# kiliant/zklaim

Hardware: AMD Instinct MI355X
Metric: Groth16 proofs/sec (zklaim gadget, alt_bn128) + G1 MSM GB/s vs HBM roofline (higher is better)
Workload: dtype u32 limbs, Montgomery (254-bit Fq/Fr: 9 x 29-bit in the accumulation, reduction and NTT kernels, 8 x 32-bit elsewhere)

## Files before the change

zklaim_amd/csrc/msm.hip:

```cpp
#include "common.hpp"
#include "fq29.hip.hpp"
#include "../../include/zkg.h"
#include <algorithm>
#include <chrono>
#include <cstdio>
#include <cstdlib>
#include <cstring>
#include <mutex>

#define ZK_VGPR_CAP(n) __attribute__((amdgpu_num_vgpr((n) / 2)))
static constexpr int ACC29_VGPRS = 192;

namespace zk {

static constexpr int SCALAR_BITS = 255;
template <class F> struct RedGeom { static constexpr int LANES_LOG = sizeof(F) == sizeof(Fq) ? 7 : 6, LANES = 1 << LANES_LOG, THREADS = 4 * LANES; };
static constexpr int RED_L_LOG_TINY = 0, RED_L_LOG_SMALL = 2, RED_L_LOG_LARGE = 4;
static constexpr size_t RED_SMALL_BUCKETS = (size_t)1 << 16, RED_LARGE_BUCKETS = (size_t)1 << 18;
static constexpr int MAX_C = 16;
static constexpr uint32_t HEAVY_S = 512;
static constexpr uint32_t HEAVY_T_MAX = 1024;
static constexpr int HEAVY_PART_BLOCKS = 512, HEAVY_MERGE_BLOCKS = 128;
static constexpr int SORT_THREADS = 1024;
static constexpr int SCAN_ITEMS = 4;

struct MsmGeom { uint32_t c, W, B, Wt, w0, ws; };
struct SetLayout { size_t buckets, items, heavy, partials, folded, red_out; };
template <class F> struct BaseView {
    const Affine<F> *p; size_t level_stride; const uint32_t *gather; uint32_t index_sub, B; const uint32_t *remap;
    template <bool PLAIN = false> ZK_D Affine<F> load(uint32_t e, size_t gb) const {
        if constexpr (PLAIN) return p[e >> 1];
        uint32_t i = e >> 1;
        if (gather) i = gather[i];
        if (remap) i = remap[i];
        if (i < index_sub) return Affine<F>::inf();
        return p[(level_stride ? (gb / B) * level_stride : 0) + (i - index_sub)];
    }
};
template <class F> struct ViewSet { BaseView<F> v[MSM_MAX_SETS]; };
struct HeavyItem { uint32_t start, end, gb, single; };
struct HeavyBucket { uint32_t gb, first_item, nparts; };

static MsmGeom pick_geom(size_t n, int window_hint, uint32_t w0 = 0, uint32_t ws = 1) {
    int lg = 0; while (((size_t)1 << (lg + 1)) <= n) ++lg;
    int c = lg >= 15 ? 16 : lg >= 11 ? 12 : lg + 1;
    if (c < 4) c = 4;
    if (window_hint > 0) c = window_hint;
    static const char *force = getenv("ZKG_MSM_C");
    if (force && atoi(force) >= 2) c = atoi(force);
    if (c > MAX_C) c = MAX_C;
    MsmGeom g; g.c = c; g.Wt = (SCALAR_BITS + c - 1) / c; g.B = 1u << (c - 1);
    g.w0 = w0; g.ws = ws ? ws : 1; g.W = w0 < g.Wt ? (g.Wt - w0 + g.ws - 1) / g.ws : 0;
    return g;
}

ZK_D uint32_t bits_at(const uint32_t v[8], uint32_t off, uint32_t c) {
    uint32_t limb = off >> 5, sh = off & 31;
    if (limb >= 8) return 0;
    uint64_t x = v[limb];
    if (limb + 1 < 8) x |= (uint64_t)v[limb + 1] << 32;
    return (uint32_t)(x >> sh) & ((1u << c) - 1);
}

ZK_D void sort_wave_priority() { __builtin_amdgcn_s_setprio(3); }


struct ZeroList { uint32_t *p[4]; uint32_t words[4]; };
__global__ __launch_bounds__(256) void k_digits(const uint32_t *scalars, const uint32_t *gather, size_t n, int mont, MsmGeom g, uint32_t *digits, ZeroList zl) {
    sort_wave_priority();
    size_t i = (size_t)blockIdx.x * blockDim.x + threadIdx.x;
    const size_t lanes = (size_t)gridDim.x * blockDim.x;
#pragma unroll
    for (int k = 0; k < 4; ++k) for (size_t z = i; z < zl.words[k]; z += lanes) zl.p[k][z] = 0;
    if (i >= n) return;
    Fr f;
    const uint4 *p = reinterpret_cast<const uint4 *>(scalars + 8 * (gather ? (size_t)gather[i] : i));
    uint4 a = p[0], b = p[1];
    f.v[0] = a.x; f.v[1] = a.y; f.v[2] = a.z; f.v[3] = a.w; f.v[4] = b.x; f.v[5] = b.y; f.v[6] = b.z; f.v[7] = b.w;
    if (mont) f = f.from_mont();
    uint32_t carry = 0;
    for (uint32_t w = 0, own = g.w0, slot = 0; w < g.Wt; ++w) {
        uint32_t raw = bits_at(f.v, w * g.c, g.c) + carry, code = 0;
        if (raw > g.B) { uint32_t d = (1u << g.c) - raw; carry = 1; if (d) code = (d << 1) | 1u; }
        else { carry = 0; if (raw) code = raw << 1; }
        if (w == own) { digits[(size_t)slot * n + i] = code; ++slot; own += g.ws; }
    }
}

template <int C>
__global__ __launch_bounds__(256) void k_digits_c(const uint32_t *scalars, const uint32_t *gather, size_t n, int mont, MsmGeom g, uint32_t *digits, ZeroList zl) {
    sort_wave_priority();
    size_t i = (size_t)blockIdx.x * blockDim.x + threadIdx.x;
    const size_t lanes = (size_t)gridDim.x * blockDim.x;
#pragma unroll
    for (int k = 0; k < 4; ++k) for (size_t z = i; z < zl.words[k]; z += lanes) zl.p[k][z] = 0;
    if (i >= n) return;
    Fr f;
    const uint4 *p = reinterpret_cast<const uint4 *>(scalars + 8 * (gather ? (size_t)gather[i] : i));
    uint4 a = p[0], b = p[1];
    f.v[0] = a.x; f.v[1] = a.y; f.v[2] = a.z; f.v[3] = a.w; f.v[4] = b.x; f.v[5] = b.y; f.v[6] = b.z; f.v[7] = b.w;
    if (mont) f = f.from_mont();
    constexpr int WT = (SCALAR_BITS + C - 1) / C;
    constexpr uint32_t B = 1u << (C - 1), MASK = (1u << C) - 1;
    uint32_t carry = 0, own = g.w0, slot = 0;
#pragma unroll
    for (int w = 0; w < WT; ++w) {
        const int off = w * C, limb = off >> 5, sh = off & 31;
        uint32_t v = limb < 8 ? f.v[limb < 8 ? limb : 7] >> sh : 0u;
        if (sh + C > 32 && limb + 1 < 8) v |= f.v[limb + 1 < 8 ? limb + 1 : 7] << (32 - sh);
        const uint32_t raw = (v & MASK) + carry;
        const bool neg = raw > B;
        const uint32_t d = neg ? (1u << C) - raw : raw;
        carry = neg ? 1u : 0u;
        const uint32_t code = d ? (d << 1) | (neg ? 1u : 0u) : 0u;
        if ((uint32_t)w == own) { digits[(size_t)slot * n + i] = code; ++slot; own += g.ws; }
    }
}

template <int C>
__global__ __launch_bounds__(256) void k_digits_multi(const uint32_t *scalars, size_t scalar_stride , size_t n, int mont, uint32_t merge, uint32_t *digits, ZeroList zl) {
    sort_wave_priority();
    size_t i = (size_t)blockIdx.x * blockDim.x + threadIdx.x;
    const size_t lanes = (size_t)gridDim.x * blockDim.x;
    if (blockIdx.y == 0) {
#pragma unroll
        for (int k = 0; k < 4; ++k) for (size_t z = i; z < zl.words[k]; z += lanes) zl.p[k][z] = 0;
    }
    if (i >= n) return;
    const uint32_t p = blockIdx.y, P = gridDim.y;
    Fr f;
    const uint4 *src = reinterpret_cast<const uint4 *>(scalars + (size_t)p * scalar_stride + 8 * i);
    uint4 a = src[0], b = src[1];
    f.v[0] = a.x; f.v[1] = a.y; f.v[2] = a.z; f.v[3] = a.w; f.v[4] = b.x; f.v[5] = b.y; f.v[6] = b.z; f.v[7] = b.w;
    if (mont) f = f.from_mont();
    constexpr int WT = (SCALAR_BITS + C - 1) / C;
    constexpr uint32_t B = 1u << (C - 1), MASK = (1u << C) - 1;
    uint32_t carry = 0;
#pragma unroll
    for (int w = 0; w < WT; ++w) {
        const int off = w * C, limb = off >> 5, sh = off & 31;
        uint32_t v = limb < 8 ? f.v[limb < 8 ? limb : 7] >> sh : 0u;
        if (sh + C > 32 && limb + 1 < 8) v |= f.v[limb + 1 < 8 ? limb + 1 : 7] << (32 - sh);
        const uint32_t raw = (v & MASK) + carry;
        const bool neg = raw > B;
        const uint32_t d = neg ? (1u << C) - raw : raw;
        carry = neg ? 1u : 0u;
        const uint32_t code = d ? (d << 1) | (neg ? 1u : 0u) : 0u;
        const size_t row = ((size_t)((uint32_t)w / merge) * P + p) * merge + (uint32_t)w % merge;
        digits[row * n + i] = code;
    }
}

__global__ __launch_bounds__(256) void k_digits_multi_any(const uint32_t *scalars, size_t scalar_stride, size_t n, int mont, MsmGeom g, uint32_t merge, uint32_t *digits, ZeroList zl) {
    sort_wave_priority();
    size_t i = (size_t)blockIdx.x * blockDim.x + threadIdx.x;
    const size_t lanes = (size_t)gridDim.x * blockDim.x;
    if (blockIdx.y == 0) {
#pragma unroll
        for (int k = 0; k < 4; ++k) for (size_t z = i; z < zl.words[k]; z += lanes) zl.p[k][z] = 0;
    }
    if (i >= n) return;
    const uint32_t p = blockIdx.y, P = gridDim.y;
    Fr f;
    const uint4 *src = reinterpret_cast<const uint4 *>(scalars + (size_t)p * scalar_stride + 8 * i);
    uint4 a = src[0], b = src[1];
    f.v[0] = a.x; f.v[1] = a.y; f.v[2] = a.z; f.v[3] = a.w; f.v[4] = b.x; f.v[5] = b.y; f.v[6] = b.z; f.v[7] = b.w;
    if (mont) f = f.from_mont();
    uint32_t carry = 0;
    for (uint32_t w = 0; w < g.Wt; ++w) {
        uint32_t raw = bits_at(f.v, w * g.c, g.c) + carry, code = 0;
        if (raw > g.B) { uint32_t d = (1u << g.c) - raw; carry = 1; if (d) code = (d << 1) | 1u; }
        else { carry = 0; if (raw) code = raw << 1; }
        const size_t row = ((size_t)(w / merge) * P + p) * merge + w % merge;
        digits[row * n + i] = code;
    }
}

template <int C>
__global__ __launch_bounds__(256) void k_digits_c4(const uint32_t *scalars, size_t n, int mont, MsmGeom g, uint32_t *digits, ZeroList zl) {
    sort_wave_priority();
    size_t i = (size_t)blockIdx.x * blockDim.x + threadIdx.x;
    const size_t lanes = (size_t)gridDim.x * blockDim.x;
#pragma unroll
    for (int k = 0; k < 4; ++k) for (size_t z = i; z < zl.words[k]; z += lanes) zl.p[k][z] = 0;
    if (4 * i >= n) return;
    Fr f[4];
#pragma unroll
    for (int q = 0; q < 4; ++q) {
        const uint4 *p = reinterpret_cast<const uint4 *>(scalars + 8 * (4 * i + q));
        const uint4 a = p[0], b = p[1];
        f[q].v[0] = a.x; f[q].v[1] = a.y; f[q].v[2] = a.z; f[q].v[3] = a.w; f[q].v[4] = b.x; f[q].v[5] = b.y; f[q].v[6] = b.z; f[q].v[7] = b.w;
        if (mont) f[q] = f[q].from_mont();
    }
    constexpr int WT = (SCALAR_BITS + C - 1) / C;
    constexpr uint32_t B = 1u << (C - 1), MASK = (1u << C) - 1;
    uint32_t carry[4] = {0, 0, 0, 0};
#pragma unroll
    for (int w = 0; w < WT; ++w) {
        const int off = w * C, limb = off >> 5, sh = off & 31;
        uint32_t code[4];
#pragma unroll
        for (int q = 0; q < 4; ++q) {
            uint32_t v = limb < 8 ? f[q].v[limb < 8 ? limb : 7] >> sh : 0u;
            if (sh + C > 32 && limb + 1 < 8) v |= f[q].v[limb + 1 < 8 ? limb + 1 : 7] << (32 - sh);
            const uint32_t raw = (v & MASK) + carry[q];
            const bool neg = raw > B;
            const uint32_t d = neg ? (1u << C) - raw : raw;
            carry[q] = neg ? 1u : 0u;
            code[q] = d ? (d << 1) | (neg ? 1u : 0u) : 0u;
        }
        *reinterpret_cast<uint4 *>(digits + (size_t)w * n + 4 * i) = make_uint4(code[0], code[1], code[2], code[3]);
    }
}

__global__ __launch_bounds__(SORT_THREADS) void k_hist(const uint32_t *digits, size_t n, uint32_t B, uint32_t S, uint32_t slice_len, uint32_t *hist) {
    extern __shared__ uint32_t lds_u32[];
    const uint32_t s = blockIdx.x, w = blockIdx.y, t = threadIdx.x;
    for (uint32_t b = t; b < B; b += SORT_THREADS) lds_u32[b] = 0;
    __syncthreads();
    size_t lo = (size_t)s * slice_len, hi = lo + slice_len < n ? lo + slice_len : n;
    const uint32_t *d = digits + (size_t)w * n;
    for (size_t i = lo + t; i < hi; i += SORT_THREADS) { uint32_t code = d[i]; if (code) atomicAdd(&lds_u32[(code >> 1) - 1], 1u); }
    __syncthreads();
    uint32_t *out = hist + ((size_t)w * S + s) * B;
    for (uint32_t b = t; b < B; b += SORT_THREADS) out[b] = lds_u32[b];
}

__global__ __launch_bounds__(256) void k_colscan(uint32_t *hist, uint32_t B, uint32_t S, size_t total, uint32_t *counts) {
    size_t gb = (size_t)blockIdx.x * blockDim.x + threadIdx.x;
    if (gb >= total) return;
    uint32_t w = (uint32_t)(gb / B), b = (uint32_t)(gb % B), run = 0;
    uint32_t *col = hist + (size_t)w * S * B + b;
    for (uint32_t s = 0; s < S; ++s) { uint32_t v = col[(size_t)s * B]; col[(size_t)s * B] = run; run += v; }
    counts[gb] = run;
}

__global__ __launch_bounds__(1024) void k_scan_blocks(const uint32_t *in, uint32_t *out, uint32_t *sums, size_t total) {
    __shared__ uint32_t part[1024];
    const uint32_t t = threadIdx.x;
    size_t base = ((size_t)blockIdx.x * 1024 + t) * SCAN_ITEMS;
    uint32_t v[SCAN_ITEMS], s = 0;
    for (int j = 0; j < SCAN_ITEMS; ++j) { v[j] = base + j < total ? in[base + j] : 0; s += v[j]; }
    part[t] = s;
    __syncthreads();
    for (uint32_t d = 1; d < 1024; d <<= 1) {
        uint32_t x = (t >= d) ? part[t - d] : 0;
        __syncthreads();
        part[t] += x;
        __syncthreads();
    }
    uint32_t run = part[t] - s;
    for (int j = 0; j < SCAN_ITEMS; ++j) { if (base + j < total) out[base + j] = run; run += v[j]; }
    if (t == 1023) sums[blockIdx.x] = part[1023];
}
__global__ __launch_bounds__(1024) void k_scan_sums(uint32_t *sums, uint32_t nblk, uint32_t *grand_total) {
    __shared__ uint32_t part[1024];
    const uint32_t t = threadIdx.x;
    uint32_t s = t < nblk ? sums[t] : 0;
    part[t] = s;
    __syncthreads();
    for (uint32_t d = 1; d < 1024; d <<= 1) {
        uint32_t x = (t >= d) ? part[t - d] : 0;
        __syncthreads();
        part[t] += x;
        __syncthreads();
    }
    if (t < nblk) sums[t] = part[t] - s;
    if (t == 1023) *grand_total = part[1023];
}
__global__ __launch_bounds__(1024) void k_scan_apply(uint32_t *out, const uint32_t *sums, size_t total) {
    size_t base = ((size_t)blockIdx.x * 1024 + threadIdx.x) * SCAN_ITEMS;
    uint32_t add = sums[blockIdx.x];
    for (int j = 0; j < SCAN_ITEMS; ++j) if (base + j < total) out[base + j] += add;
}

__global__ __launch_bounds__(SORT_THREADS) void k_place(const uint32_t *digits, size_t n, uint32_t B, uint32_t S, uint32_t slice_len,
                                                         const uint32_t *hist, const uint32_t *offsets, uint32_t *sorted) {
    extern __shared__ uint32_t lds_u32[];
    const uint32_t s = blockIdx.x, w = blockIdx.y, t = threadIdx.x;
    const uint32_t *rel = hist + ((size_t)w * S + s) * B, *off = offsets + (size_t)w * B;
    for (uint32_t b = t; b < B; b += SORT_THREADS) lds_u32[b] = off[b] + rel[b];
    __syncthreads();
    size_t lo = (size_t)s * slice_len, hi = lo + slice_len < n ? lo + slice_len : n;
    const uint32_t *d = digits + (size_t)w * n;
    for (size_t i = lo + t; i < hi; i += SORT_THREADS) {
        uint32_t code = d[i];
        if (code) { uint32_t pos = atomicAdd(&lds_u32[(code >> 1) - 1], 1u); sorted[pos] = ((uint32_t)i << 1) | (code & 1u); }
    }
}


static constexpr uint32_t RX_MAX_CBITS = 10, RX_MAX_CB = 1u << RX_MAX_CBITS, RX_SLICE = 16384, RX_PER_THREAD = 16, RX_FINE_MAX = 8192, RX_BIN_AVG = 4096;
__global__ __launch_bounds__(1024) void k_rx_count(const uint32_t *digits, size_t n, uint32_t fbits, uint32_t cbits, uint32_t *cnt) {
    sort_wave_priority();
    __shared__ uint32_t c[RX_MAX_CB];
    const uint32_t sl = blockIdx.x, w = blockIdx.y, t = threadIdx.x, CB = 1u << cbits;
    if (t < CB) c[t] = 0;
    __syncthreads();
    size_t lo = (size_t)sl * RX_SLICE, hi = lo + RX_SLICE < n ? lo + RX_SLICE : n;
    const uint32_t *d = digits + (size_t)w * n;
    if ((n & 3) == 0) {
        for (size_t i = lo + 4 * t; i < hi; i += 4096) {
            const uint4 q = *reinterpret_cast<const uint4 *>(d + i);
            if (q.x) atomicAdd(&c[((q.x >> 1) - 1) >> fbits], 1u);
            if (q.y) atomicAdd(&c[((q.y >> 1) - 1) >> fbits], 1u);
            if (q.z) atomicAdd(&c[((q.z >> 1) - 1) >> fbits], 1u);
            if (q.w) atomicAdd(&c[((q.w >> 1) - 1) >> fbits], 1u);
        }
    } else
    for (size_t i = lo + t; i < hi; i += 1024) { uint32_t code = d[i]; if (code) atomicAdd(&c[((code >> 1) - 1) >> fbits], 1u); }
    __syncthreads();
    if (t < CB && c[t]) atomicAdd(&cnt[w * CB + t], c[t]);
}
__global__ __launch_bounds__(1024) void k_rx_scan(const uint32_t *cnt, uint32_t nbins, uint32_t *base, uint32_t *cursor, uint32_t *grand_total) {
    sort_wave_priority();
    __shared__ uint32_t part[1024];
    const uint32_t t = threadIdx.x, per = (nbins + 1023) / 1024, lo = t * per, hi = lo + per < nbins ? lo + per : nbins;
    uint32_t sum = 0;
    for (uint32_t i = lo; i < hi; ++i) sum += cnt[i];
    part[t] = sum;
    __syncthreads();
    for (uint32_t d = 1; d < 1024; d <<= 1) {
        uint32_t x = (t >= d) ? part[t - d] : 0;
        __syncthreads();
        part[t] += x;
        __syncthreads();
    }
    uint32_t run = part[t] - sum;
    for (uint32_t i = lo; i < hi; ++i) { base[i] = run; cursor[i] = 0; run += cnt[i]; }
    if (t == 1023) { base[nbins] = part[1023]; *grand_total = part[1023]; }
}
template <int T>
__global__ __launch_bounds__(T) void k_rx_scatter(const uint32_t *digits, size_t n, uint32_t fbits, uint32_t cbits, const uint32_t *base, uint32_t *cursor,
                                                   uint32_t *tmp) {
    sort_wave_priority();
    extern __shared__ uint32_t lds_u32[];
    constexpr uint32_t SLICE = RX_PER_THREAD * T;
    const uint32_t CB = 1u << cbits;
    uint32_t *stage = lds_u32, *c = lds_u32 + SLICE, *off = c + RX_MAX_CB, *gb = off + RX_MAX_CB + 1, *cur = gb + RX_MAX_CB;
    const uint32_t sl = blockIdx.x, w = blockIdx.y, t = threadIdx.x;
    for (uint32_t b = t; b < CB; b += T) c[b] = 0;
    __syncthreads();
    size_t lo = (size_t)sl * SLICE, hi = lo + SLICE < n ? lo + SLICE : n;
    const uint32_t *d = digits + (size_t)w * n;
    uint32_t code[RX_PER_THREAD];
    const bool vec = (n & 3) == 0;
    auto elem = [&](uint32_t j) -> size_t { return vec ? lo + 4 * (size_t)t + (size_t)(j >> 2) * (4 * T) + (j & 3) : lo + t + (size_t)j * T; };
    if (vec) {
#pragma unroll
        for (uint32_t j = 0; j < RX_PER_THREAD; j += 4) {
            const size_t i = elem(j);
            uint4 q = make_uint4(0, 0, 0, 0);
            if (i < hi) q = *reinterpret_cast<const uint4 *>(d + i);
            code[j] = q.x; code[j + 1] = q.y; code[j + 2] = q.z; code[j + 3] = q.w;
        }
    } else {
#pragma unroll
        for (uint32_t j = 0; j < RX_PER_THREAD; ++j) { const size_t i = elem(j); code[j] = i < hi ? d[i] : 0; }
    }
#pragma unroll
    for (uint32_t j = 0; j < RX_PER_THREAD; ++j) if (code[j]) atomicAdd(&c[((code[j] >> 1) - 1) >> fbits], 1u);
    __syncthreads();
    const uint32_t b0 = t, b1 = t + T;
    if (b0 < CB) off[b0] = c[b0];
    if (b1 < CB) off[b1] = c[b1];
    __syncthreads();
    for (uint32_t dd = 1; dd < CB; dd <<= 1) {
        const uint32_t x0 = (b0 < CB && b0 >= dd) ? off[b0 - dd] : 0, x1 = (b1 < CB && b1 >= dd) ? off[b1 - dd] : 0;
        __syncthreads();
        if (b0 < CB) off[b0] += x0;
        if (b1 < CB) off[b1] += x1;
        __syncthreads();
    }
    if (t == 0) off[CB] = off[CB - 1];
    __syncthreads();
    for (uint32_t b = t; b < CB; b += T) { off[b] -= c[b]; gb[b] = c[b] ? base[w * CB + b] + atomicAdd(&cursor[w * CB + b], c[b]) : 0; cur[b] = 0; }
    __syncthreads();
    const uint32_t fmask = (1u << fbits) - 1;
#pragma unroll
    for (uint32_t j = 0; j < RX_PER_THREAD; ++j) {
        if (!code[j]) continue;
        uint32_t i = (uint32_t)elem(j), b = (code[j] >> 1) - 1, k = b >> fbits;
        uint32_t pos = off[k] + atomicAdd(&cur[k], 1u);
        stage[pos] = ((b & fmask) << (32 - fbits)) | (i << 1) | (code[j] & 1u);
    }
    __syncthreads();
    const uint32_t wave = t >> 6, lane = t & 63;
    for (uint32_t k = wave; k < CB; k += T / 64) {
        const uint32_t a = off[k], b = off[k + 1], g = gb[k];
        for (uint32_t p = a + lane; p < b; p += 64) tmp[g + (p - a)] = stage[p];
    }
}
ZK_D void rx_fine_offsets(uint32_t *cf, uint32_t *of, uint32_t FB, uint32_t t, uint32_t start, size_t gb0, uint32_t *counts, uint32_t *offsets) {
    const uint32_t T = blockDim.x;
    if (t < FB) of[t] = cf[t];
    __syncthreads();
    for (uint32_t d = 1; d < FB; d <<= 1) {
        uint32_t x = (t < FB && t >= d) ? of[t - d] : 0;
        __syncthreads();
        if (t < FB) of[t] += x;
        __syncthreads();
    }
    if (t < FB) of[t] -= cf[t];
    __syncthreads();
    for (uint32_t f = t; f < FB; f += T) { counts[gb0 + f] = cf[f]; offsets[gb0 + f] = start + of[f]; }
}
ZK_D void rx_fine_big_bin(const uint32_t *tmp, uint32_t fbits, uint32_t start, uint32_t cnt, size_t gb0, uint32_t *cf, uint32_t *of, uint32_t *cur, uint32_t *counts,
                          uint32_t *offsets, uint32_t *sorted) {
    const uint32_t FB = 1u << fbits, sh = 32 - fbits, low = (1u << sh) - 1, t = threadIdx.x, T = blockDim.x;
    const bool giant = cnt > 8 * RX_FINE_MAX;
    if (!giant) {
        for (uint32_t p = t; p < cnt; p += T) atomicAdd(&cf[tmp[start + p] >> sh], 1u);
    } else
    for (uint32_t p0 = 0; p0 < cnt; p0 += T) {
        uint32_t p = p0 + t; bool live = p < cnt; uint32_t f = live ? tmp[start + p] >> sh : 0;
        while (__any(live)) {
            uint32_t lf = __shfl(f, __ffsll((long long)__ballot(live)) - 1, 64);
            unsigned long long same = __ballot(live && f == lf);
            if (live && f == lf) { if ((same & ((1ull << (threadIdx.x & 63)) - 1)) == 0) atomicAdd(&cf[lf], (uint32_t)__popcll(same)); live = false; }
        }
    }
    __syncthreads();
    rx_fine_offsets(cf, of, FB, t, start, gb0, counts, offsets);
    if (!giant) {
        for (uint32_t p = t; p < cnt; p += T) { uint32_t e = tmp[start + p], f = e >> sh; sorted[start + of[f] + atomicAdd(&cur[f], 1u)] = e & low; }
        return;
    }
    for (uint32_t p0 = 0; p0 < cnt; p0 += T) {
        uint32_t p = p0 + t; bool live = p < cnt; uint32_t e = live ? tmp[start + p] : 0, f = e >> sh;
        while (__any(live)) {
            uint32_t lf = __shfl(f, __ffsll((long long)__ballot(live)) - 1, 64);
            unsigned long long same = __ballot(live && f == lf), below = same & ((1ull << (threadIdx.x & 63)) - 1);
            uint32_t basepos = 0;
            if (live && f == lf && below == 0) basepos = atomicAdd(&cur[lf], (uint32_t)__popcll(same));
            basepos = __shfl(basepos, __ffsll((long long)same) - 1, 64);
            if (live && f == lf) { sorted[start + of[lf] + basepos + (uint32_t)__popcll(below)] = e & low; live = false; }
        }
    }
}
template <int T>
__global__ __launch_bounds__(T) void k_rx_fine(const uint32_t *tmp, uint32_t fbits, uint32_t cbits, uint32_t B, const uint32_t *base, uint32_t *counts, uint32_t *offsets,
                                                uint32_t *sorted) {
    sort_wave_priority();
    extern __shared__ uint32_t lds_u32[];
    const uint32_t FB = 1u << fbits, sh = 32 - fbits, low = (1u << sh) - 1;
    uint32_t *bufB = lds_u32, *cf = bufB + RX_FINE_MAX, *of = cf + FB, *cur = of + FB;
    const uint32_t cb = blockIdx.x, w = blockIdx.y, t = threadIdx.x, bin = (w << cbits) + cb;
    const uint32_t start = base[bin], cnt = base[bin + 1] - start;
    const size_t gb0 = (size_t)w * B + (size_t)cb * FB;
    for (uint32_t f = t; f < FB; f += T) { cf[f] = 0; cur[f] = 0; }
    __syncthreads();
    if (cnt > RX_FINE_MAX) { rx_fine_big_bin(tmp, fbits, start, cnt, gb0, cf, of, cur, counts, offsets, sorted); return; }
    uint32_t ent[RX_FINE_MAX / T];
#pragma unroll
    for (uint32_t j = 0; j < RX_FINE_MAX / T; ++j) {
        uint32_t p = t + j * T;
        ent[j] = p < cnt ? tmp[start + p] : 0xffffffffu;
        if (p < cnt) atomicAdd(&cf[ent[j] >> sh], 1u);
    }
    __syncthreads();
    rx_fine_offsets(cf, of, FB, t, start, gb0, counts, offsets);
#pragma unroll
    for (uint32_t j = 0; j < RX_FINE_MAX / T; ++j) {
        if (t + j * T >= cnt) continue;
        uint32_t e = ent[j], f = e >> sh;
        bufB[of[f] + atomicAdd(&cur[f], 1u)] = e & low;
    }
    __syncthreads();
    for (uint32_t p = t; p < cnt; p += T) sorted[start + p] = bufB[p];
}

ZK_D uint32_t heavy_threshold_dev(const uint32_t *offsets, size_t total_buckets, uint32_t divisor) {
    uint32_t entries = offsets[total_buckets];
    uint32_t avg6 = (uint32_t)(6 * (uint64_t)entries / total_buckets), slack = 8 + avg6 > 32 ? 32 : 8 + avg6;
    uint32_t t = (uint32_t)(4 * (uint64_t)entries / total_buckets) + slack;
    t = t > HEAVY_T_MAX ? HEAVY_T_MAX : t;
    t /= divisor;
    return t < 4 ? 4 : t;
}

__global__ __launch_bounds__(1024) void k_class_hist(const uint32_t *counts, const uint32_t *offsets, size_t total, uint32_t *class_hist) {
    sort_wave_priority();
    __shared__ uint32_t h[HEAVY_T_MAX + 2];
    const uint32_t heavy_t = heavy_threshold_dev(offsets, total, 1);
    const uint32_t t = threadIdx.x, nc = heavy_t + 2;
    for (uint32_t i = t; i < nc; i += 1024) h[i] = 0;
    __syncthreads();
    size_t gb = (size_t)blockIdx.x * 1024 + t;
    if (gb < total) { uint32_t c = counts[gb]; atomicAdd(&h[c > heavy_t ? heavy_t + 1 : c], 1u); }
    __syncthreads();
    for (uint32_t i = t; i < nc; i += 1024) if (h[i]) atomicAdd(&class_hist[i], h[i]);
}
__global__ __launch_bounds__(1024) void k_class_scan(uint32_t *class_hist, const uint32_t *offsets, size_t total) {
    sort_wave_priority();
    __shared__ uint32_t part[1024];
    const uint32_t heavy_t = heavy_threshold_dev(offsets, total, 1), nc = heavy_t + 2, t = threadIdx.x;
    uint32_t v0 = 2 * t < nc ? class_hist[nc - 1 - 2 * t] : 0, v1 = 2 * t + 1 < nc ? class_hist[nc - 2 - 2 * t] : 0;
    part[t] = v0 + v1;
    __syncthreads();
    for (uint32_t d = 1; d < 1024; d <<= 1) {
        uint32_t x = (t >= d) ? part[t - d] : 0;
        __syncthreads();
        part[t] += x;
        __syncthreads();
    }
    const uint32_t before = part[t] - v0 - v1;
    if (2 * t < nc) class_hist[nc - 1 - 2 * t] = before;
    if (2 * t + 1 < nc) class_hist[nc - 2 - 2 * t] = before + v0;
}
__global__ __launch_bounds__(1024) void k_order_place(const uint32_t *counts, const uint32_t *offsets, size_t total, uint32_t *class_cursor, uint32_t *order) {
    sort_wave_priority();
    __shared__ uint32_t h[HEAVY_T_MAX + 2];
    const uint32_t heavy_t = heavy_threshold_dev(offsets, total, 1);
    const uint32_t t = threadIdx.x, nc = heavy_t + 2;
    for (uint32_t i = t; i < nc; i += 1024) h[i] = 0;
    __syncthreads();
    size_t gb = (size_t)blockIdx.x * 1024 + t;
    uint32_t cls = 0, rank = 0;
    if (gb < total) { uint32_t c = counts[gb]; cls = c > heavy_t ? heavy_t + 1 : c; rank = atomicAdd(&h[cls], 1u); }
    __syncthreads();
    for (uint32_t i = t; i < nc; i += 1024) if (h[i]) h[i] = atomicAdd(&class_cursor[i], h[i]);
    __syncthreads();
    if (gb < total) order[h[cls] + rank] = (uint32_t)gb;
}

template <class F, bool PLAIN>
__global__ __launch_bounds__(256) void k_bucket_accum(const ViewSet<F> views, const uint32_t *sorted, const uint32_t *offsets, const uint32_t *order,
                                                       size_t lanes , XYZZ<F> *buckets, HeavyItem *items,
                                                       HeavyBucket *heavy, uint32_t *counters , SetLayout L) {
    size_t tid = (size_t)blockIdx.x * blockDim.x + threadIdx.x;
    if (tid >= lanes) return;
    const size_t total_buckets = L.buckets;
    const uint32_t set = blockIdx.y;
    const BaseView<F> bases = views.v[set];
    buckets += set * L.buckets; items += set * L.items; heavy += set * L.heavy; counters += 2 * set;
    const uint32_t heavy_t = heavy_threshold_dev(offsets, total_buckets, sizeof(F) > sizeof(Fq) ? 3 : 1);
    const uint32_t gb = order[tid];
    uint32_t k = offsets[gb], end = offsets[gb + 1];
    if (end - k > heavy_t) {
        uint32_t nparts = (end - k + HEAVY_S - 1) / HEAVY_S;
        uint32_t first = atomicAdd(&counters[0], nparts);
        for (uint32_t p = 0; p < nparts; ++p) { uint32_t a = k + p * HEAVY_S; items[first + p] = {a, a + HEAVY_S < end ? a + HEAVY_S : end, gb, nparts == 1}; }
        if (nparts > 1) heavy[atomicAdd(&counters[1], 1u)] = {gb, first, nparts};
        return;
    }
    XYZZ<F> acc = XYZZ<F>::inf();
    if (k < end) {
        uint32_t e = sorted[k], e_next = k + 1 < end ? sorted[k + 1] : 0;
        Affine<F> p = bases.template load<PLAIN>(e, gb);
        while (true) {
            Affine<F> cur = p; uint32_t ce = e;
            ++k;
            if (k < end) { e = e_next; p = bases.template load<PLAIN>(e, gb); if (k + 1 < end) e_next = sorted[k + 1]; }
            if (ce & 1u) cur.y = cur.y.neg();
            acc.madd(cur);
            if (k >= end) break;
        }
    }
    buckets[gb] = acc.normalized();
}

__global__ __launch_bounds__(256) void k_bases_to29(const Affine<Fq> *in, size_t n, Rec64 *out) {
    size_t i = (size_t)blockIdx.x * blockDim.x + threadIdx.x;
    if (i >= n) return;
    const Affine<Fq> a = in[i];
    store_rec64(out + i, f29::to29(a.x), f29::to29(a.y), a.is_inf());
}
ZK_D Affine29 load29(const Rec64 *bases, uint32_t e) { return load_rec64(bases + (e >> 1)); }
ZK_D Rec64 load29_raw(const Rec64 *bases, uint32_t e) { return load_rec64_raw(bases + (e >> 1)); }
template <int WAVES, bool OUT29>
__global__ __launch_bounds__(256, WAVES) ZK_VGPR_CAP(ACC29_VGPRS) void k_bucket_accum29(const Rec64 *bases, size_t level_stride, uint32_t B, const uint32_t *sorted, const uint32_t *offsets, const uint32_t *order,
                                                         size_t lanes, void *buckets_, HeavyItem *items, HeavyBucket *heavy, uint32_t *counters, SetLayout L, int flags ) {
    crit_wave_priority(flags & 2);
    const int resume = flags & 1;
    size_t tid = (size_t)blockIdx.x * blockDim.x + threadIdx.x;
    if (tid >= lanes) return;
    const uint32_t heavy_t = heavy_threshold_dev(offsets, L.buckets, 1);
    const uint32_t gb = order[tid];
    if (level_stride) bases += (size_t)(gb / B) * level_stride;
    uint32_t k = offsets[gb], end = offsets[gb + 1];
    if (end - k > heavy_t) {
        uint32_t nparts = (end - k + HEAVY_S - 1) / HEAVY_S;
        uint32_t first = atomicAdd(&counters[0], nparts);
        const bool single = nparts == 1 && !resume;
        for (uint32_t p = 0; p < nparts; ++p) { uint32_t a = k + p * HEAVY_S; items[first + p] = {a, a + HEAVY_S < end ? a + HEAVY_S : end, gb, single}; }
        if (!single) heavy[atomicAdd(&counters[1], 1u)] = {gb, first, nparts};
        return;
    }
    XYZZ29 acc; bool inf = true;
    acc.x = acc.y = acc.zz = acc.zzz = Fq29::zero();
    if constexpr (OUT29) {
        if (resume) {
            if (k >= end) return;
            const Bucket29 old = load_bucket29_raw(reinterpret_cast<const Bucket29 *>(buckets_) + gb);
            uint32_t any = 0;
#pragma unroll
            for (int j = 0; j < 9; ++j) { acc.x.v[j] = old.x[j]; acc.y.v[j] = old.y[j]; acc.zz.v[j] = old.zz[j]; acc.zzz.v[j] = old.zzz[j]; any |= old.zz[j]; }
            inf = any == 0;
        }
    }
    if (k < end) {
        uint32_t e = sorted[k], e_next = k + 1 < end ? sorted[k + 1] : 0;
        Rec64 p = load29_raw(bases, e);
        while (true) {
            const Rec64 curw = p; const uint32_t ce = e;
            ++k;
            if (k < end) { e = e_next; p = load29_raw(bases, e); if (k + 1 < end) e_next = sorted[k + 1]; }
            const Affine29 cur = unpack_rec64(curw);
            if (!cur.inf) {
                Fq29 bx, by;
#pragma unroll
                for (int j = 0; j < 9; ++j) { bx.v[j] = cur.x[j]; by.v[j] = cur.y[j]; }
                if (ce & 1u) by = f29::neg(f29::S2_1, by);
                if (__builtin_expect(!acc.madd(bx, by, inf), 0)) {
                    XYZZ<Fq> a32 = {f29::from29(acc.x), f29::from29(acc.y), f29::from29(acc.zz), f29::from29(acc.zzz)};
                    a32.madd(Affine<Fq>{f29::from29(bx), f29::from29(f29::norm(by))});
                    if (a32.is_inf()) inf = true;
                    else { acc.x = f29::to29(a32.x.normalized()); acc.y = f29::to29(a32.y.normalized()); acc.zz = f29::to29(a32.zz.normalized()); acc.zzz = f29::to29(a32.zzz.normalized()); }
                }
            }
            if (k >= end) break;
        }
    }
    if constexpr (OUT29) store_bucket29(reinterpret_cast<Bucket29 *>(buckets_) + gb, acc, inf);
    else {
        XYZZ<Fq> *buckets = reinterpret_cast<XYZZ<Fq> *>(buckets_);
        if (inf) buckets[gb] = XYZZ<Fq>::inf().normalized();
        else buckets[gb] = XYZZ<Fq>{f29::from29(acc.x), f29::from29(acc.y), f29::from29(acc.zz), f29::from29(acc.zzz)};
    }
}

template <class F> struct alignas(16) LdsPoint {
    XYZZ<F> p; uint32_t pad[4];
    ZK_D LdsPoint &operator=(const XYZZ<F> &v) { p = v; return *this; }
    ZK_D operator const XYZZ<F> &() const { return p; }
    ZK_D XYZZ<F> normalized() const { return p.normalized(); }
};

template <class F, class Barrier>
ZK_D void lds_tree_reduce(LdsPoint<F> *seg, uint32_t n, uint32_t tid, uint32_t nthreads, Barrier barrier) {
    for (uint32_t d = n / 2; d >= 1; d >>= 1) {
        if (4 * d <= nthreads) {
            uint32_t t = tid >> 2, q = tid & 3;
            if (t < d) { XYZZ<F> a = seg[t]; xyzz_add_quad(a, seg[t + d].p, q); if (q == 0) seg[t] = a; }
        } else if (tid < d) { XYZZ<F> a = seg[tid]; a.add(seg[tid + d]); seg[tid] = a; }
        barrier();
    }
}

template <class F> ZK_D void put_bucket(XYZZ<F> *buckets, uint32_t gb, const XYZZ<F> &v, int out29) {
    if constexpr (sizeof(F) == sizeof(Fq)) { if (out29) { store_bucket29(reinterpret_cast<Bucket29 *>(buckets) + gb, v); return; } }
    buckets[gb] = v;
}
template <class F>
__global__ __launch_bounds__(256) void k_heavy_parts(const ViewSet<F> views, const uint32_t *sorted, const HeavyItem *items,
                                                      const uint32_t *counters, XYZZ<F> *partials, XYZZ<F> *buckets, SetLayout L, int out29) {
    extern __shared__ unsigned char red_smem[];
    LdsPoint<F> *sh = reinterpret_cast<LdsPoint<F> *>(red_smem);
    const uint32_t set = blockIdx.y;
    const BaseView<F> bases = views.v[set];
    items += set * L.items; partials += set * L.partials; buckets += set * L.buckets;
    const uint32_t n_items = counters[2 * set], t = threadIdx.x, lane = t & 63, wv = t >> 6;
    for (uint32_t base = blockIdx.x * 4; base < n_items; base += gridDim.x * 4) {
        uint32_t it = base + wv;
        XYZZ<F> acc = XYZZ<F>::inf();
        if (it < n_items) {
            HeavyItem h = items[it];
            for (uint32_t k = h.start + lane; k < h.end; k += 64) {
                uint32_t e = sorted[k];
                Affine<F> p = bases.load(e, h.gb);
                if (e & 1u) p.y = p.y.neg();
                acc.madd(p);
            }
        }
        sh[t] = acc;
        __syncthreads();
        lds_tree_reduce<F>(sh + wv * 64, 64, lane, 64, [] { __syncthreads(); });
        if (lane == 0 && it < n_items) { if (items[it].single) put_bucket<F>(buckets, items[it].gb, sh[t].normalized(), out29); else partials[it] = sh[t].normalized(); }
        __syncthreads();
    }
}

template <class F>
__global__ __launch_bounds__(256) void k_heavy_merge(const HeavyBucket *heavy, const uint32_t *counters, const XYZZ<F> *partials, XYZZ<F> *buckets, SetLayout L, int out29, int resume) {
    extern __shared__ unsigned char red_smem[];
    LdsPoint<F> *sh = reinterpret_cast<LdsPoint<F> *>(red_smem);
    const uint32_t set = blockIdx.y;
    heavy += set * L.heavy; partials += set * L.partials; buckets += set * L.buckets;
    const uint32_t n_heavy = counters[2 * set + 1], t = threadIdx.x;
    for (uint32_t hb = blockIdx.x; hb < n_heavy; hb += gridDim.x) {
        HeavyBucket h = heavy[hb];
        XYZZ<F> acc = XYZZ<F>::inf();
        for (uint32_t p = t; p < h.nparts; p += 256) acc.add(partials[h.first_item + p]);
        if constexpr (sizeof(F) == sizeof(Fq)) {
            if (resume && out29 && t == 255) acc.add(bucket29_to_xyzz(load_bucket29_raw(reinterpret_cast<const Bucket29 *>(buckets) + h.gb)));
        }
        sh[t] = acc;
        __syncthreads();
        lds_tree_reduce<F>(sh, 256, t, 256, [] { __syncthreads(); });
        if (t == 0) put_bucket<F>(buckets, h.gb, sh[0].normalized(), out29);
        __syncthreads();
    }
}

template <class F, int RED_L_LOG>
__global__ __launch_bounds__(RedGeom<F>::THREADS) void k_bucket_reduce(const XYZZ<F> *buckets, uint32_t B, uint32_t chunks_per_window, XYZZ<F> *out,
                                                                       size_t in_set_stride, size_t out_set_stride) {
    constexpr int RED_LANES = RedGeom<F>::LANES, RED_L = 1 << RED_L_LOG, RED_CHUNK = RED_LANES * RED_L;
    extern __shared__ unsigned char red_smem[];
    LdsPoint<F> *sh = reinterpret_cast<LdsPoint<F> *>(red_smem);
    const uint32_t t = threadIdx.x >> 2, q = threadIdx.x & 3;
    const uint32_t w = blockIdx.x / chunks_per_window, ch = blockIdx.x % chunks_per_window;
    const XYZZ<F> *X = buckets + blockIdx.y * in_set_stride + (size_t)w * B;
    out += blockIdx.y * out_set_stride;
    const uint32_t base = ch * RED_CHUNK + t * RED_L;
    XYZZ<F> run = XYZZ<F>::inf(), T0 = XYZZ<F>::inf();
    XYZZ<F> cur = (base + RED_L - 1 < B) ? X[base + RED_L - 1] : XYZZ<F>::inf();
    for (int j = RED_L - 1; j >= 1; --j) {
        XYZZ<F> nxt = (base + j - 1 < B) ? X[base + j - 1] : XYZZ<F>::inf();
        xyzz_add_quad(run, cur, q);
        xyzz_add_quad(T0, run, q);
        cur = nxt;
    }
    xyzz_add_quad(run, cur, q);
    XYZZ<F> Q = run;
    for (uint32_t d = 1; d < RED_LANES; d <<= 1) {
        if (q == 0) sh[t] = Q;
        __syncthreads();
        if (t + d < RED_LANES) xyzz_add_quad(Q, sh[t + d].p, q);
        __syncthreads();
    }
    XYZZ<F> P = Q;
    if (q == 0) { sh[t] = (t >= 1) ? Q : XYZZ<F>::inf(); sh[RED_LANES + t] = T0; }
    __syncthreads();
    for (uint32_t d = RED_LANES / 2; d >= 1; d >>= 1) {
        if (t < d) { XYZZ<F> a = sh[t]; xyzz_add_quad(a, sh[t + d].p, q); if (q == 0) sh[t] = a; }
        else if (t >= RED_LANES / 2 && t < RED_LANES / 2 + d) {
            uint32_t u = RED_LANES + (t - RED_LANES / 2);
            XYZZ<F> a = sh[u]; xyzz_add_quad(a, sh[u + d].p, q); if (q == 0) sh[u] = a;
        }
        __syncthreads();
    }
    if (t == 0) {
        XYZZ<F> E = sh[0];
        for (int i = 0; i < RED_L_LOG; ++i) E = E.dbl();
        xyzz_add_quad(E, sh[RED_LANES].p, q);
        if (q == 0) { out[2 * (size_t)blockIdx.x] = P.normalized(); out[2 * (size_t)blockIdx.x + 1] = E.normalized(); }
    }
}

struct alignas(16) LdsPoint29 { XYZZ29q p; uint32_t pad[4]; };
template <bool IN29> ZK_D XYZZ29q load_bucket29(const void *X_, uint32_t i, uint32_t B, uint32_t q) {
    if (i >= B) return XYZZ29q::inf();
    if constexpr (IN29) {
        const Bucket29 b = load_bucket29_raw(reinterpret_cast<const Bucket29 *>(X_) + i);
        XYZZ29q r;
#pragma unroll
        for (int j = 0; j < 9; ++j) { r.x.v[j] = b.x[j]; r.y.v[j] = b.y[j]; r.zz.v[j] = b.zz[j]; r.zzz.v[j] = b.zzz[j]; }
        return r;
    } else {
        const XYZZ<Fq> b = reinterpret_cast<const XYZZ<Fq> *>(X_)[i];
        if (b.is_inf()) return XYZZ29q::inf();
        return quad_load29(b.x, b.y, b.zz, b.zzz, q);
    }
}
ZK_D XYZZ<Fq> store_point29(const XYZZ29q &p) {
    if (p.is_inf()) return XYZZ<Fq>::inf().normalized();
    return {f29::from29(p.x), f29::from29(p.y), f29::from29(p.zz), f29::from29(p.zzz)};
}
template <int RED_L_LOG, bool IN29>
__global__ __launch_bounds__(RedGeom<Fq>::THREADS) void k_bucket_reduce29(const void *buckets, uint32_t B, uint32_t chunks_per_window, XYZZ<Fq> *out,
                                                                          size_t in_set_stride, size_t out_set_stride, int critical) {
    crit_wave_priority(critical);
    constexpr int RED_LANES = RedGeom<Fq>::LANES, RED_L = 1 << RED_L_LOG, RED_CHUNK = RED_LANES * RED_L;
    extern __shared__ unsigned char red_smem[];
    LdsPoint29 *sh = reinterpret_cast<LdsPoint29 *>(red_smem);
    const uint32_t t = threadIdx.x >> 2, q = threadIdx.x & 3;
    const uint32_t w = blockIdx.x / chunks_per_window, ch = blockIdx.x % chunks_per_window;
    const size_t elem = IN29 ? sizeof(Bucket29) : sizeof(XYZZ<Fq>);
    const void *X = reinterpret_cast<const char *>(buckets) + (blockIdx.y * in_set_stride + (size_t)w * B) * elem;
    out += blockIdx.y * out_set_stride;
    const uint32_t base = ch * RED_CHUNK + t * RED_L;
    XYZZ29q run = XYZZ29q::inf(), T0 = XYZZ29q::inf();
    XYZZ29q cur = load_bucket29<IN29>(X, base + RED_L - 1, B, q);
    for (int j = RED_L - 1; j >= 1; --j) {
        const XYZZ29q nxt = load_bucket29<IN29>(X, base + j - 1, B, q);
        xyzz29_add_quad(run, cur, q);
        xyzz29_add_quad(T0, run, q);
        cur = nxt;
    }
    xyzz29_add_quad(run, cur, q);
    XYZZ29q Q = run;
    for (uint32_t d = 1; d < RED_LANES; d <<= 1) {
        if (q == 0) sh[t].p = Q;
        __syncthreads();
        if (t + d < RED_LANES) xyzz29_add_quad(Q, sh[t + d].p, q);
        __syncthreads();
    }
    const XYZZ29q P = Q;
    if (q == 0) { sh[t].p = (t >= 1) ? Q : XYZZ29q::inf(); sh[RED_LANES + t].p = T0; }
    __syncthreads();
    for (uint32_t d = RED_LANES / 2; d >= 1; d >>= 1) {
        if (t < d) { XYZZ29q a = sh[t].p; xyzz29_add_quad(a, sh[t + d].p, q); if (q == 0) sh[t].p = a; }
        else if (t >= RED_LANES / 2 && t < RED_LANES / 2 + d) {
            const uint32_t u = RED_LANES + (t - RED_LANES / 2);
            XYZZ29q a = sh[u].p; xyzz29_add_quad(a, sh[u + d].p, q); if (q == 0) sh[u].p = a;
        }
        __syncthreads();
    }
    if (t == 0) {
        XYZZ<Fq> E = store_point29(sh[0].p);
        for (int i = 0; i < RED_L_LOG; ++i) E = E.dbl();
        E.add(store_point29(sh[RED_LANES].p));
        if (q == 0) { out[2 * (size_t)blockIdx.x] = store_point29(P); out[2 * (size_t)blockIdx.x + 1] = E.normalized(); }
    }
}

ZK_D Half29 lds_load_half29(const LdsPoint29 *p, uint32_t r) {
    const uint32_t *w = reinterpret_cast<const uint32_t *>(p) + 9 * r;
    Half29 h;
#pragma unroll
    for (int i = 0; i < 9; ++i) { h.c0.v[i] = w[i]; h.c1.v[i] = w[18 + i]; }
    return h;
}
ZK_D void lds_store_half29(LdsPoint29 *p, const Half29 &h, uint32_t r) {
    uint32_t *w = reinterpret_cast<uint32_t *>(p) + 9 * r;
#pragma unroll
    for (int i = 0; i < 9; ++i) { w[i] = h.c0.v[i]; w[18 + i] = h.c1.v[i]; }
}
template <bool IN29> ZK_D Half29 load_half29(const void *X_, uint32_t i, uint32_t B, uint32_t r) {
    if (i >= B) return Half29::inf();
    if constexpr (IN29) {
        const uint32_t *w = reinterpret_cast<const uint32_t *>(reinterpret_cast<const Bucket29 *>(X_) + i) + 9 * r;
        Half29 h;
#pragma unroll
        for (int j = 0; j < 9; ++j) { h.c0.v[j] = w[j]; h.c1.v[j] = w[18 + j]; }
        return h;
    } else {
        const Fq *f = reinterpret_cast<const Fq *>(reinterpret_cast<const XYZZ<Fq> *>(X_) + i);
        const Fq c0 = f[r], c1 = f[2 + r];
        if (c1.is_zero()) return Half29::inf();
        Fq29 to; for (int j = 0; j < 9; ++j) to.v[j] = f29::TO[j];
        Half29 h; f29::mul2(h.c0, h.c1, f29::unpack(c0), to, f29::unpack(c1), to);
        return h;
    }
}
template <int RED_L_LOG, bool IN29>
__global__ __launch_bounds__(2 * RedGeom<Fq>::LANES) void k_bucket_reduce29p(const void *buckets, uint32_t B, uint32_t chunks_per_window, XYZZ<Fq> *out,
                                                                             size_t in_set_stride, size_t out_set_stride, int critical) {
    crit_wave_priority(critical);
    constexpr int RED_LANES = RedGeom<Fq>::LANES, RED_L = 1 << RED_L_LOG, RED_CHUNK = RED_LANES * RED_L;
    extern __shared__ unsigned char red_smem[];
    LdsPoint29 *sh = reinterpret_cast<LdsPoint29 *>(red_smem);
    const uint32_t t = threadIdx.x >> 1, r = threadIdx.x & 1;
    const uint32_t w = blockIdx.x / chunks_per_window, ch = blockIdx.x % chunks_per_window;
    const size_t elem = IN29 ? sizeof(Bucket29) : sizeof(XYZZ<Fq>);
    const void *X = reinterpret_cast<const char *>(buckets) + (blockIdx.y * in_set_stride + (size_t)w * B) * elem;
    out += blockIdx.y * out_set_stride;
    const uint32_t base = ch * RED_CHUNK + t * RED_L;
    Half29 run = Half29::inf(), T0 = Half29::inf();
    Half29 cur = load_half29<IN29>(X, base + RED_L - 1, B, r);
    for (int j = RED_L - 1; j >= 1; --j) {
        const Half29 nxt = load_half29<IN29>(X, base + j - 1, B, r);
        xyzz29_add_pair(run, cur, r);
        xyzz29_add_pair(T0, run, r);
        cur = nxt;
    }
    xyzz29_add_pair(run, cur, r);
    Half29 Q = run;
    for (uint32_t d = 1; d < RED_LANES; d <<= 1) {
        lds_store_half29(sh + t, Q, r);
        __syncthreads();
        if (t + d < RED_LANES) xyzz29_add_pair(Q, lds_load_half29(sh + t + d, r), r);
        __syncthreads();
    }
    const Half29 P = Q;
    lds_store_half29(sh + t, t >= 1 ? Q : Half29::inf(), r); lds_store_half29(sh + RED_LANES + t, T0, r);
    __syncthreads();
    for (uint32_t d = RED_LANES / 2; d >= 1; d >>= 1) {
        if (t < d) { Half29 a = lds_load_half29(sh + t, r); xyzz29_add_pair(a, lds_load_half29(sh + t + d, r), r); lds_store_half29(sh + t, a, r); }
        else if (t >= RED_LANES / 2 && t < RED_LANES / 2 + d) {
            const uint32_t u = RED_LANES + (t - RED_LANES / 2);
            Half29 a = lds_load_half29(sh + u, r); xyzz29_add_pair(a, lds_load_half29(sh + u + d, r), r); lds_store_half29(sh + u, a, r);
        }
        __syncthreads();
    }
    if (t == 0) lds_store_half29(sh + 1, P, r);
    __syncthreads();
    if (threadIdx.x == 0) {
        XYZZ<Fq> E = store_point29(sh[0].p);
        for (int i = 0; i < RED_L_LOG; ++i) E = E.dbl();
        E.add(store_point29(sh[RED_LANES].p));
        out[2 * (size_t)blockIdx.x] = store_point29(sh[1].p); out[2 * (size_t)blockIdx.x + 1] = E.normalized();
    }
}

__global__ __launch_bounds__(2 * RedGeom<Fq>::LANES) void k_bucket_reduce29l(const Bucket29 *buckets, uint32_t B, uint32_t chunks_per_window, XYZZ<Fq> *out,
                                                                             size_t in_set_stride, size_t out_set_stride, int critical) {
    crit_wave_priority(critical);
    constexpr int RED_LANES = RedGeom<Fq>::LANES, NT = 2 * RED_LANES, PER = 8, RED_CHUNK = NT * PER;
    static_assert(RED_CHUNK == (RED_LANES << RED_L_LOG_LARGE), "the lane-form reduction keeps the large reduction's chunks");
    extern __shared__ unsigned char red_smem[];
    LdsPoint29 *sh = reinterpret_cast<LdsPoint29 *>(red_smem);
    const uint32_t i = threadIdx.x;
    const uint32_t w = blockIdx.x / chunks_per_window, ch = blockIdx.x % chunks_per_window;
    const Bucket29 *X = buckets + blockIdx.y * in_set_stride + (size_t)w * B;
    out += blockIdx.y * out_set_stride;
    {
        const uint32_t base = ch * RED_CHUNK + i * PER;
        XYZZ29q run = XYZZ29q::inf(), T0 = XYZZ29q::inf();
        XYZZ29q cur = load_bucket29<true>(X, base + PER - 1, B, 0);
        for (int j = PER - 1; j >= 1; --j) {
            const XYZZ29q nxt = load_bucket29<true>(X, base + j - 1, B, 0);
            xyzz29_add_lane(run, cur);
            xyzz29_add_lane(T0, run);
            cur = nxt;
        }
        xyzz29_add_lane(run, cur);
        sh[i].p = run; sh[NT + i].p = T0;
    }
    __syncthreads();
    const uint32_t t = i >> 1, r = i & 1;
    const Half29 R1 = lds_load_half29(sh + 2 * t + 1, r);
    Half29 Q = lds_load_half29(sh + 2 * t, r);
    xyzz29_add_pair(Q, R1, r);
    Half29 Tp = lds_load_half29(sh + NT + 2 * t, r);
    xyzz29_add_pair(Tp, lds_load_half29(sh + NT + 2 * t + 1, r), r);
    __syncthreads();
    for (uint32_t d = 1; d < RED_LANES; d <<= 1) {
        lds_store_half29(sh + t, Q, r);
        __syncthreads();
        if (t + d < RED_LANES) xyzz29_add_pair(Q, lds_load_half29(sh + t + d, r), r);
        __syncthreads();
    }
    const Half29 P = Q;
    lds_store_half29(sh + t, Q, r);
    __syncthreads();
    Half29 V = t + 1 < RED_LANES ? lds_load_half29(sh + t + 1, r) : Half29::inf();
    xyzz29_add_pair(V, R1, r);
    if (t >= 1) xyzz29_add_pair(V, Q, r);
    __syncthreads();
    lds_store_half29(sh + t, V, r); lds_store_half29(sh + RED_LANES + t, Tp, r);
    __syncthreads();
    for (uint32_t d = RED_LANES / 2; d >= 1; d >>= 1) {
        if (t < d) { Half29 a = lds_load_half29(sh + t, r); xyzz29_add_pair(a, lds_load_half29(sh + t + d, r), r); lds_store_half29(sh + t, a, r); }
        else if (t >= RED_LANES / 2 && t < RED_LANES / 2 + d) {
            const uint32_t u = RED_LANES + (t - RED_LANES / 2);
            Half29 a = lds_load_half29(sh + u, r); xyzz29_add_pair(a, lds_load_half29(sh + u + d, r), r); lds_store_half29(sh + u, a, r);
        }
        __syncthreads();
    }
    if (t == 0) lds_store_half29(sh + 1, P, r);
    __syncthreads();
    if (threadIdx.x < 3) out[3 * (size_t)blockIdx.x + threadIdx.x] = store_point29(threadIdx.x == 0 ? sh[1].p : threadIdx.x == 1 ? sh[RED_LANES].p : sh[0].p);
}


__global__ __launch_bounds__(256) void k_bucket_fold29(const Bucket29 *buckets, const uint32_t *counts, uint32_t W, uint32_t B, Bucket29 *out, int critical) {
    crit_wave_priority(critical);
    const uint32_t b = (blockIdx.x * blockDim.x + threadIdx.x) >> 1, r = threadIdx.x & 1;
    if (b >= B) return;
    Half29 acc = Half29::inf();
    uint32_t w = 0;
    while (w < W && !counts[(size_t)w * B + b]) ++w;
    Half29 cur = w < W ? load_half29<true>(buckets + (size_t)w * B, b, B, r) : Half29::inf();
    while (w < W) {
        uint32_t nw = w + 1;
        while (nw < W && !counts[(size_t)nw * B + b]) ++nw;
        const Half29 nxt = nw < W ? load_half29<true>(buckets + (size_t)nw * B, b, B, r) : Half29::inf();
        xyzz29_add_pair(acc, cur, r);
        cur = nxt; w = nw;
    }
    uint32_t *o = reinterpret_cast<uint32_t *>(out + b) + 9 * r;
#pragma unroll
    for (int i = 0; i < 9; ++i) { o[i] = acc.c0.v[i]; o[18 + i] = acc.c1.v[i]; }
}

static constexpr uint32_t FOLD_THREADS = 256;
template <class F>
__global__ __launch_bounds__(FOLD_THREADS) void k_bucket_fold(const XYZZ<F> *buckets, const uint32_t *counts, uint32_t W, uint32_t B, uint32_t fold_b_log, XYZZ<F> *out, SetLayout L) {
    extern __shared__ unsigned char red_smem[];
    LdsPoint<F> *sh = reinterpret_cast<LdsPoint<F> *>(red_smem);
    const uint32_t t = threadIdx.x, FB = 1u << fold_b_log, slots = FOLD_THREADS >> fold_b_log;
    const uint32_t bl = t & (FB - 1), slot = t >> fold_b_log, b = blockIdx.x * FB + bl;
    buckets += blockIdx.y * L.buckets; out += blockIdx.y * L.folded;
    XYZZ<F> acc = XYZZ<F>::inf();
    if (b < B) for (uint32_t w = slot; w < W; w += slots) if (counts[(size_t)w * B + b]) acc.add(buckets[(size_t)w * B + b]);
    sh[t] = acc;
    __syncthreads();
    for (uint32_t d = slots / 2; d >= 1; d >>= 1) {
        const uint32_t pairs = d << fold_b_log;
        if (4 * pairs <= FOLD_THREADS) {
            const uint32_t u = t >> 2, q = t & 3;
            if (u < pairs) { XYZZ<F> a = sh[u]; xyzz_add_quad(a, sh[u + pairs].p, q); if (q == 0) sh[u] = a; }
        } else if (t < pairs) { XYZZ<F> a = sh[t]; a.add(sh[t + pairs]); sh[t] = a; }
        __syncthreads();
    }
    if (t < FB && b < B) out[b] = sh[t].normalized();
}

template <class F> ZK_D F inverse_fast(const F &x) {
    if constexpr (std::is_same<F, Fq>::value) return f29::from29(f29::inverse(f29::to29(x.normalized())));
    else { const Fq d = inverse_fast<Fq>(x.c0.sqr() + x.c1.sqr()); return F{x.c0 * d, (x.c1 * d).neg()}; }
}
template <class F, int K>
__global__ __launch_bounds__(256) void k_table_levels(const Affine<F> *in, Affine<F> *out, size_t n, uint32_t c, int levels) {
    size_t i = (size_t)blockIdx.x * blockDim.x + threadIdx.x;
    if (i >= n) return;
    Affine<F> a = in[i];
    if (a.is_inf()) { for (int l = 0; l < levels; ++l) out[(size_t)l * n + i] = a; return; }
    F x[K], y[K], zz[K], zzz[K];
    XYZZ<F> p = XYZZ<F>::dbl_affine_inl(a);
#pragma unroll
    for (int l = 0; l < K; ++l) {
        if (l < levels) {
            for (uint32_t k = (l == 0 ? 1u : 0u); k < c; ++k) p = p.dbl();
            x[l] = p.x; y[l] = p.y; zz[l] = p.zz; zzz[l] = p.zzz;
        } else { x[l] = F::zero(); y[l] = F::zero(); zz[l] = F::zero(); zzz[l] = F::zero(); }
    }
    F pre[K], run = F::one();
#pragma unroll
    for (int l = 0; l < K; ++l) { pre[l] = run; if (!zzz[l].is_zero()) run = run * zzz[l]; }
    F inv = inverse_fast(run);
#pragma unroll
    for (int l = K - 1; l >= 0; --l) {
        if (l >= levels) continue;
        if (zzz[l].is_zero()) { out[(size_t)l * n + i] = Affine<F>::inf(); continue; }
        F zi = inv * pre[l];
        inv = inv * zzz[l];
        F t = zi * zz[l];
        F zi2 = t.sqr();
        out[(size_t)l * n + i] = Affine<F>{x[l] * zi2, y[l] * zi}.normalized();
    }
}

__global__ __launch_bounds__(256) void k_classify(const Fr *z, size_t n1, uint8_t *tags, uint32_t *listed, uint32_t *count, const uint32_t *subset_pos) {
    size_t i = (size_t)blockIdx.x * blockDim.x + threadIdx.x;
    uint32_t tag = 0;
    if (i < n1) {
        Fr v = z[i];
        uint32_t any = 0, diff = 0;
#pragma unroll
        for (int j = 0; j < 8; ++j) { any |= v.v[j]; diff |= v.v[j] ^ FrParams::ONE[j]; }
        tag = any == 0 ? 0u : (diff == 0 ? 1u : 2u);
        tags[i] = (uint8_t)tag;
    }
    const unsigned long long mask = __ballot(tag == 2);
    if (!mask) return;
    const uint32_t lane = threadIdx.x & 63;
    uint32_t base = 0;
    if (lane == (uint32_t)(__ffsll((long long)mask) - 1)) base = atomicAdd(count, (uint32_t)__popcll(mask));
    base = __shfl(base, __ffsll((long long)mask) - 1, 64);
    if (tag == 2) {
        listed[base + (uint32_t)__popcll(mask & ((1ull << lane) - 1))] = (uint32_t)i;
        if (subset_pos && subset_pos[i] == SUBSET_NONE) count[1] = 1;
    }
}
template <class F>
__global__ __launch_bounds__(256) void k_gather_points(const Affine<F> *src, const uint32_t *idx, size_t count, uint32_t index_sub, Affine<F> *out) {
    size_t j = (size_t)blockIdx.x * blockDim.x + threadIdx.x;
    if (j >= count) return;
    const uint32_t i = idx[j];
    out[j] = i >= index_sub ? src[i - index_sub] : Affine<F>::inf();
}
template <class F>
__global__ __launch_bounds__(256) void k_scatter_points(const Affine<F> *src, const uint32_t *idx, size_t count, Affine<F> *out) {
    size_t j = (size_t)blockIdx.x * blockDim.x + threadIdx.x;
    if (j < count) out[idx[j]] = src[j];
}
template <class F>
__global__ __launch_bounds__(256) void k_ones_sum(const ViewSet<F> views, const uint8_t *tags, size_t n1, uint32_t span, XYZZ<F> *partials,
                                                   size_t tag_stride, size_t vec_stride ) {
    extern __shared__ unsigned char red_smem[];
    LdsPoint<F> *sh = reinterpret_cast<LdsPoint<F> *>(red_smem);
    uint32_t *list = reinterpret_cast<uint32_t *>(red_smem + 256 * sizeof(LdsPoint<F>));
    __shared__ uint32_t seg_count[4];
    const Affine<F> *bases = views.v[blockIdx.y].p; const uint32_t index_sub = views.v[blockIdx.y].index_sub;
    tags += (size_t)blockIdx.z * tag_stride;
    partials += (size_t)blockIdx.z * vec_stride + (size_t)blockIdx.y * (gridDim.x + 1);
    const uint32_t tid = threadIdx.x, lane = tid & 63, wv = tid >> 6, cap = span >> 2;
    const size_t first = (size_t)blockIdx.x * span + (size_t)wv * cap;
    uint32_t count = 0;
    for (uint32_t o = 0; o < cap; o += 64) {
        const size_t i = first + o + lane;
        const bool one = i < n1 && i >= index_sub && tags[i] == 1;
        const unsigned long long mask = __ballot(one);
        if (one) list[wv * cap + count + (uint32_t)__popcll(mask & ((1ull << lane) - 1))] = (uint32_t)(i - index_sub);
        count += (uint32_t)__popcll(mask);
    }
    if (lane == 0) seg_count[wv] = count;
    __syncthreads();
    const uint32_t c0 = seg_count[0], c1 = c0 + seg_count[1], c2 = c1 + seg_count[2], total = c2 + seg_count[3];
    XYZZ<F> acc = XYZZ<F>::inf();
    for (uint32_t k = tid; k < total; k += 256) {
        const uint32_t seg = (k >= c0) + (k >= c1) + (k >= c2), off = seg == 0 ? 0u : (seg == 1 ? c0 : (seg == 2 ? c1 : c2));
        acc.madd(bases[list[seg * cap + (k - off)]]);
    }
    sh[tid] = acc;
    __syncthreads();
    lds_tree_reduce<F>(sh, 256, tid, 256, [] { __syncthreads(); });
    if (tid == 0) partials[blockIdx.x] = sh[0].normalized();
}
template <class F>
__global__ __launch_bounds__(256) void k_sum_partials(XYZZ<F> *partials_all, uint32_t count, size_t vec_stride) {
    extern __shared__ unsigned char red_smem[];
    LdsPoint<F> *sh = reinterpret_cast<LdsPoint<F> *>(red_smem);
    XYZZ<F> *partials = partials_all + (size_t)blockIdx.y * vec_stride + (size_t)blockIdx.x * (count + 1), *out = partials + count;
    XYZZ<F> acc = XYZZ<F>::inf();
    for (uint32_t i = threadIdx.x; i < count; i += 256) acc.add(partials[i]);
    sh[threadIdx.x] = acc;
    __syncthreads();
    lds_tree_reduce<F>(sh, 256, threadIdx.x, 256, [] { __syncthreads(); });
    if (threadIdx.x == 0) out[0] = sh[0].normalized();
}

struct MsmGroup {
    DevBuf buckets, folded, red_out, heavy_items, heavy_buckets, heavy_counters, heavy_partials;
    DevBuf bases29;
    void *host_red = nullptr; size_t host_cap = 0; bool g2 = false, table = false; int nsets = 0;
    int out_index[MSM_MAX_SETS] = {0};
    int red_slots = 2; size_t red_stride = 0;
    uint32_t cpw = 0, red_windows = 0; size_t nred = 0; int chunk_log = 0;
    int host_reserve(size_t bytes) {
        if (bytes <= host_cap) return 0;
        if (host_red) (void)hipHostFree(host_red);
        host_red = nullptr; host_cap = 0;
        if (!hip_ok(hipHostMalloc(&host_red, bytes + 4096, hipHostMallocDefault), "hipHostMalloc", __FILE__, __LINE__)) return 1;
        host_cap = bytes + 4096;
        return 0;
    }
    void release() {
        for (DevBuf *b : {&buckets, &folded, &red_out, &heavy_items, &heavy_buckets, &heavy_counters, &heavy_partials, &bases29}) b->release();
        if (host_red) (void)hipHostFree(host_red);
        host_red = nullptr; host_cap = 0;
    }
};
struct MsmJob {
    hipStream_t stream = nullptr; bool own_stream = false;
    DevBuf digits, hist, counts, offsets, scan_sums, class_hist, order, sorted, rx_tmp, rx_meta;
    MsmGroup group[2];
    MsmGeom g{}; size_t n = 0;
    int window_hint = 0;
    uint32_t merge_hint = 1, merge = 1;
    hipStream_t aux = nullptr; hipEvent_t ev_fork = nullptr, ev_join = nullptr; bool converted_aside = false;
    bool one_pass_sort = false;
    bool resume = false, defer_reduce = false;
    bool critical = false;
    MsmJob *bucket_owner = nullptr;
    hipStream_t sort_stream = nullptr; hipEvent_t ev_sorted = nullptr, ev_acc_done = nullptr;
    uint32_t w0 = 0, ws = 1;
    bool empty = false;
    bool dev_finish = false;
    uint32_t multi = 1; size_t multi_stride = 0;
    DevBuf hs_scalars; hipStream_t copy = nullptr; hipEvent_t ev_piece[8] = {nullptr};
    std::mutex mu;
};

template <class F>
static int launch_accumulate(MsmJob *job, MsmGroup &gr, const MsmBases *sets, const uint32_t *d_gather, bool time_it) {
    const MsmGeom g = job->g; const size_t n = job->n, total_buckets = (size_t)g.W * g.B; const unsigned ns = (unsigned)gr.nsets;
    const uint32_t P = job->multi, BP = g.B * P, Wp = g.W / P;
    hipStream_t s = job->stream;
    size_t n_entries_max = n * g.W;
    const size_t max_heavy = std::min(total_buckets, n_entries_max / (sizeof(F) != sizeof(Fq) ? 4 : 8)) + 1,
                 max_items = max_heavy + n_entries_max / HEAVY_S + 1;
    typedef RedGeom<F> RG;
    gr.table = sets[0].level_stride != 0;
    gr.red_windows = gr.table ? P : g.W;
    const size_t red_buckets = (size_t)gr.red_windows * g.B;
    static const char *force_l = getenv("ZKG_RED_L_LOG");
    const int red_l_log = force_l ? atoi(force_l) : red_buckets >= RED_LARGE_BUCKETS ? RED_L_LOG_LARGE : red_buckets > RED_SMALL_BUCKETS ? RED_L_LOG_SMALL : RED_L_LOG_TINY;
    gr.chunk_log = RG::LANES_LOG + red_l_log;
    gr.cpw = (g.B + (1u << gr.chunk_log) - 1) >> gr.chunk_log; gr.nred = (size_t)gr.red_windows * gr.cpw;
    DevBuf &bucket_buf = job->bucket_owner ? job->bucket_owner->group[sizeof(F) != sizeof(Fq) ? 1 : 0].buckets : gr.buckets;
    gr.red_slots = 2;
    SetLayout L; L.buckets = total_buckets; L.items = max_items; L.heavy = max_heavy; L.partials = max_items; L.folded = BP; L.red_out = gr.nred * 3;
    if (gr.heavy_items.reserve(ns * max_items * sizeof(HeavyItem)) || gr.heavy_buckets.reserve(ns * max_heavy * sizeof(HeavyBucket)) ||
        gr.heavy_counters.reserve(8 * MSM_MAX_SETS) || gr.heavy_partials.reserve(ns * max_items * sizeof(XYZZ<F>)) ||
        bucket_buf.reserve(ns * total_buckets * std::max(sizeof(XYZZ<F>), sizeof(Bucket29))) || gr.red_out.reserve(ns * L.red_out * sizeof(XYZZ<F>)) || ((gr.red_stride = L.red_out), false) ||
        (gr.table && gr.folded.reserve(ns * (size_t)BP * std::max(sizeof(XYZZ<F>), sizeof(Bucket29)))) || (!job->dev_finish && gr.host_reserve(ns * L.red_out * sizeof(XYZZ<F>)))) return ZKG_ERROR;
    XYZZ<F> *buckets = bucket_buf.as<XYZZ<F>>();
    ViewSet<F> views;
    for (unsigned i = 0; i < (unsigned)MSM_MAX_SETS; ++i) {
        const MsmBases &b = sets[i < ns ? i : 0];
        views.v[i] = BaseView<F>{reinterpret_cast<const Affine<F> *>(b.p), b.level_stride, d_gather, b.index_sub, BP, b.remap};
    }
    const size_t lanes = gr.table ? std::min(total_buckets, n_entries_max) : total_buckets;
    bool plain = !d_gather;
    for (unsigned i = 0; i < ns; ++i) plain = plain && sets[i].level_stride == 0 && sets[i].index_sub == 0 && !sets[i].remap;
    bool use29 = false; const Rec64 *rec29 = nullptr; size_t stride29 = 0;
    if constexpr (sizeof(F) == sizeof(Fq)) {
        if (ns == 1 && plain) {
            use29 = true;
            if (sets[0].p29) rec29 = reinterpret_cast<const Rec64 *>(sets[0].p29);
            else {
                ZK_HIP(hipStreamWaitEvent(s, job->ev_join, 0));
                rec29 = gr.bases29.as<Rec64>();
            }
        } else if (ns == 1 && !d_gather && sets[0].p29 && !sets[0].remap && sets[0].index_sub == 0) {
            use29 = true; rec29 = reinterpret_cast<const Rec64 *>(sets[0].p29); stride29 = sets[0].level_stride;
        }
    }
    const bool out29 = use29 && (stride29 == 0 ? !gr.table : (gr.table && ns == 1 && Wp <= 8));
    const int resume = job->resume ? 1 : 0;
    if (time_it) g_dominant_timer.begin(s);
    if constexpr (sizeof(F) == sizeof(Fq)) {
        static const int waves_env = getenv("ZKG_ACC29_WAVES") ? atoi(getenv("ZKG_ACC29_WAVES")) : 0;
        const int waves29 = waves_env ? waves_env : (job->sort_stream || gr.table || job->bucket_owner) ? 2 : 3;
        auto launch29 = [&](auto kern) {
            hipLaunchKernelGGL(kern, dim3((unsigned)((lanes + 255) / 256)), dim3(256), 0, s, rec29, stride29, BP, job->sorted.as<uint32_t>(),
                               job->offsets.as<uint32_t>(), job->order.as<uint32_t>(), lanes, (void *)buckets, gr.heavy_items.as<HeavyItem>(),
                               gr.heavy_buckets.as<HeavyBucket>(), gr.heavy_counters.as<uint32_t>(), L, resume | (job->critical ? 2 : 0));
        };
        if (use29 && waves29 == 3) { if (out29) launch29(k_bucket_accum29<3, true>); else launch29(k_bucket_accum29<3, false>); }
        else if (use29) { if (out29) launch29(k_bucket_accum29<2, true>); else launch29(k_bucket_accum29<2, false>); }
    }
    if (use29) {}
    else if (plain)
        hipLaunchKernelGGL((k_bucket_accum<F, true>), dim3((unsigned)((lanes + 255) / 256), ns), dim3(256), 0, s,
                           views, job->sorted.as<uint32_t>(), job->offsets.as<uint32_t>(), job->order.as<uint32_t>(), lanes, buckets,
                           gr.heavy_items.as<HeavyItem>(), gr.heavy_buckets.as<HeavyBucket>(), gr.heavy_counters.as<uint32_t>(), L);
    else
        hipLaunchKernelGGL((k_bucket_accum<F, false>), dim3((unsigned)((lanes + 255) / 256), ns), dim3(256), 0, s,
                           views, job->sorted.as<uint32_t>(), job->offsets.as<uint32_t>(), job->order.as<uint32_t>(), lanes, buckets,
                           gr.heavy_items.as<HeavyItem>(), gr.heavy_buckets.as<HeavyBucket>(), gr.heavy_counters.as<uint32_t>(), L);
    if (time_it) g_dominant_timer.end(s);
    hipLaunchKernelGGL(k_heavy_parts<F>, dim3(HEAVY_PART_BLOCKS, ns), dim3(256), 256 * sizeof(LdsPoint<F>), s,
                       views, job->sorted.as<uint32_t>(), gr.heavy_items.as<HeavyItem>(), gr.heavy_counters.as<uint32_t>(), gr.heavy_partials.as<XYZZ<F>>(), buckets, L, (int)out29);
    hipLaunchKernelGGL(k_heavy_merge<F>, dim3(HEAVY_MERGE_BLOCKS, ns), dim3(256), 256 * sizeof(LdsPoint<F>), s,
                       gr.heavy_buckets.as<HeavyBucket>(), gr.heavy_counters.as<uint32_t>(), gr.heavy_partials.as<XYZZ<F>>(), buckets, L, (int)out29, resume);
    if (job->defer_reduce) {
        if (hipGetLastError() != hipSuccess) { set_error("msm kernel launch failed"); return ZKG_ERROR; }
        return ZKG_OK;
    }
    const XYZZ<F> *red_in = buckets; size_t in_stride = L.buckets;
    bool folded29 = false;
    if constexpr (sizeof(F) == sizeof(Fq)) {
        if (gr.table && out29) {
            hipLaunchKernelGGL(k_bucket_fold29, dim3((2 * BP + 255) / 256), dim3(256), 0, s, reinterpret_cast<const Bucket29 *>(buckets), job->counts.as<uint32_t>(), Wp, BP,
                               gr.folded.as<Bucket29>(), job->critical ? 1 : 0);
            red_in = gr.folded.as<XYZZ<F>>(); in_stride = L.folded; folded29 = true;
        }
    }
    if (gr.table && !folded29) {
        uint32_t slots = 1; while (slots < Wp && slots < 32) slots <<= 1;
        uint32_t fold_b_log = 0; while ((FOLD_THREADS >> (fold_b_log + 1)) >= slots) ++fold_b_log;
        hipLaunchKernelGGL(k_bucket_fold<F>, dim3((BP + (1u << fold_b_log) - 1) >> fold_b_log, ns), dim3(FOLD_THREADS), FOLD_THREADS * sizeof(LdsPoint<F>), s,
                           buckets, job->counts.as<uint32_t>(), Wp, BP, fold_b_log, gr.folded.as<XYZZ<F>>(), L);
        red_in = gr.folded.as<XYZZ<F>>(); in_stride = L.folded;
    }
    if constexpr (sizeof(F) == sizeof(Fq)) {
        const size_t lds = 2 * RG::LANES * sizeof(LdsPoint29);
        const void *rin = red_in; XYZZ<Fq> *rout = reinterpret_cast<XYZZ<Fq> *>(gr.red_out.p);
        auto launch_red = [&](auto kern, unsigned threads) { hipLaunchKernelGGL(kern, dim3((unsigned)gr.nred, ns), dim3(threads), lds, s, rin, g.B, gr.cpw, rout, in_stride, L.red_out, job->critical ? 1 : 0); };
        if (out29 && red_l_log == RED_L_LOG_LARGE) {
            gr.red_slots = 3;
            hipLaunchKernelGGL(k_bucket_reduce29l, dim3((unsigned)gr.nred, ns), dim3(2 * RG::LANES), 4 * RG::LANES * sizeof(LdsPoint29), s,
                               reinterpret_cast<const Bucket29 *>(rin), g.B, gr.cpw, rout, in_stride, L.red_out, job->critical ? 1 : 0);
        } else if (red_l_log != RED_L_LOG_TINY) {
            if (red_l_log == RED_L_LOG_LARGE) launch_red(k_bucket_reduce29p<RED_L_LOG_LARGE, false>, 2 * RG::LANES);
            else if (out29) launch_red(k_bucket_reduce29p<RED_L_LOG_SMALL, true>, 2 * RG::LANES);
            else launch_red(k_bucket_reduce29p<RED_L_LOG_SMALL, false>, 2 * RG::LANES);
        } else {
            if (out29) launch_red(k_bucket_reduce29<RED_L_LOG_TINY, true>, RG::THREADS);
            else launch_red(k_bucket_reduce29<RED_L_LOG_TINY, false>, RG::THREADS);
        }
    } else {
        if (red_l_log == RED_L_LOG_LARGE)
            hipLaunchKernelGGL((k_bucket_reduce<F, RED_L_LOG_LARGE>), dim3((unsigned)gr.nred, ns), dim3(RG::THREADS), 2 * RG::LANES * sizeof(LdsPoint<F>), s,
                               red_in, g.B, gr.cpw, gr.red_out.as<XYZZ<F>>(), in_stride, L.red_out);
        else if (red_l_log == RED_L_LOG_SMALL)
            hipLaunchKernelGGL((k_bucket_reduce<F, RED_L_LOG_SMALL>), dim3((unsigned)gr.nred, ns), dim3(RG::THREADS), 2 * RG::LANES * sizeof(LdsPoint<F>), s,
                               red_in, g.B, gr.cpw, gr.red_out.as<XYZZ<F>>(), in_stride, L.red_out);
        else
            hipLaunchKernelGGL((k_bucket_reduce<F, RED_L_LOG_TINY>), dim3((unsigned)gr.nred, ns), dim3(RG::THREADS), 2 * RG::LANES * sizeof(LdsPoint<F>), s,
                               red_in, g.B, gr.cpw, gr.red_out.as<XYZZ<F>>(), in_stride, L.red_out);
    }
    if (hipGetLastError() != hipSuccess) { set_error("msm kernel launch failed"); return ZKG_ERROR; }
    if (job->dev_finish) return ZKG_OK;
    ZK_HIP(hipMemcpyAsync(gr.host_red, gr.red_out.p, ns * L.red_out * sizeof(XYZZ<F>), hipMemcpyDeviceToHost, s));
    return ZKG_OK;
}

template <class F>
static XYZZ<F> host_combine(const MsmJob *job, const MsmGroup &gr, int set, int vec = 0 ) {
    const MsmGeom g = job->g; const uint32_t cpw = gr.cpw, W = gr.red_windows;
    const bool multi = gr.table && job->multi > 1;
    const XYZZ<F> *red = reinterpret_cast<const XYZZ<F> *>(gr.host_red) + (size_t)set * gr.red_stride;
    const size_t sl = (size_t)gr.red_slots;
    std::vector<XYZZ<F>> V(W);
    auto window = [&](int w) {
        XYZZ<F> Usum = XYZZ<F>::inf(), suffix = XYZZ<F>::inf(), weighted = XYZZ<F>::inf(), Asum = XYZZ<F>::inf();
        for (int ch = (int)cpw - 1; ch >= 0; --ch) {
            const XYZZ<F> &P = red[sl * ((size_t)w * cpw + ch)], &U = red[sl * ((size_t)w * cpw + ch) + 1];
            Usum.add(U);
            if (sl == 3) Asum.add(red[sl * ((size_t)w * cpw + ch) + 2]);
            if (ch >= 1) { suffix.add(P); weighted.add(suffix); }
            else suffix.add(P);
        }
        if (sl == 3 && !Asum.is_inf()) { for (int i = 0; i < 3; ++i) Asum = Asum.dbl(); Usum.add(Asum); }
        if (!weighted.is_inf()) for (int i = 0; i < gr.chunk_log; ++i) weighted = weighted.dbl();
        Usum.add(weighted); Usum.add(suffix);
        V[w] = Usum;
    };
    if (multi) { window(vec); return V[vec]; }
    if (gr.table) {
        const int SEG = 16, nseg = ((int)cpw + SEG - 1) / SEG;
        if (nseg <= 1) { window(0); return V[0]; }
        std::vector<XYZZ<F>> Us(nseg), Ps(nseg), Wt(nseg);
        host_parallel_for(nseg, [&](int sg) {
            XYZZ<F> Usum = XYZZ<F>::inf(), suffix = XYZZ<F>::inf(), weighted = XYZZ<F>::inf();
            const int lo = sg * SEG, hi = std::min<int>((int)cpw, lo + SEG);
            for (int ch = hi - 1; ch >= lo; --ch) {
                Usum.add(red[2 * (size_t)ch + 1]);
                suffix.add(red[2 * (size_t)ch]);
                if (ch > lo) weighted.add(suffix);
            }
            Us[sg] = Usum; Ps[sg] = suffix; Wt[sg] = weighted;
        });
        XYZZ<F> Usum = XYZZ<F>::inf(), suffix = XYZZ<F>::inf(), seg_weighted = XYZZ<F>::inf(), weighted = XYZZ<F>::inf();
        for (int sg = nseg - 1; sg >= 0; --sg) { Usum.add(Us[sg]); weighted.add(Wt[sg]); suffix.add(Ps[sg]); if (sg >= 1) seg_weighted.add(suffix); }
        if (!seg_weighted.is_inf()) for (int i = 0; i < 4; ++i) seg_weighted = seg_weighted.dbl();
        weighted.add(seg_weighted);
        if (!weighted.is_inf()) for (int i = 0; i < gr.chunk_log; ++i) weighted = weighted.dbl();
        Usum.add(weighted); Usum.add(suffix);
        return Usum;
    }
    host_parallel_for((int)W, window);
    XYZZ<F> acc = XYZZ<F>::inf();
    for (int w = (int)W - 1; w >= 0; --w) {
        if (!acc.is_inf()) for (uint32_t i = 0; i < g.c * g.ws; ++i) acc = acc.dbl();
        acc.add(V[w]);
    }
    if (!acc.is_inf()) for (uint32_t i = 0; i < g.c * g.w0; ++i) acc = acc.dbl();
    return acc;
}

static constexpr int COMBINE_THREADS = 256;
ZK_D void store_norm_dev(uint32_t *out , const XYZZ<Fq> &v) {
    Fq X = Fq::zero(), Y = Fq::one(), Z = Fq::zero();
    if (!v.is_inf()) { const Affine<Fq> a = v.to_affine().normalized(); X = a.x; Y = a.y; Z = Fq::one(); }
    for (int i = 0; i < 8; ++i) { out[i] = X.v[i]; out[8 + i] = Y.v[i]; out[16 + i] = Z.v[i]; }
}
__global__ __launch_bounds__(COMBINE_THREADS) void k_msm_combine(const XYZZ<Fq> *red, uint32_t cpw, int slots, int chunk_log, size_t set_stride, uint32_t *out) {
    extern __shared__ unsigned char red_smem[];
    LdsPoint<Fq> *sh = reinterpret_cast<LdsPoint<Fq> *>(red_smem);
    const uint32_t t = threadIdx.x, w = blockIdx.x, set = blockIdx.y;
    uint32_t n = 1; while (n < cpw && n < (uint32_t)COMBINE_THREADS) n <<= 1;
    int l_log = 0; while (((uint64_t)n << l_log) < cpw) ++l_log;
    const XYZZ<Fq> *rec = red + (size_t)set * set_stride + (size_t)slots * w * cpw;
    const uint64_t first = (uint64_t)t << l_log, end = first + ((uint64_t)1 << l_log) < cpw ? first + ((uint64_t)1 << l_log) : cpw;
    XYZZ<Fq> U = XYZZ<Fq>::inf(), S = XYZZ<Fq>::inf(), T0 = XYZZ<Fq>::inf(), A = XYZZ<Fq>::inf();
    for (uint64_t ch = end; ch > first; --ch) {
        const XYZZ<Fq> *r = rec + (size_t)slots * (ch - 1);
        S.add(r[0]); U.add(r[1]);
        if (slots == 3) A.add(r[2]);
        if (ch - 1 > first) T0.add(S);
    }
    XYZZ<Fq> Q = S;
    for (uint32_t d = 1; d < n; d <<= 1) {
        if (t < n) sh[t] = Q;
        __syncthreads();
        if (t + d < n) Q.add(sh[t + d]);
        __syncthreads();
    }
    XYZZ<Fq> Wt = t >= 1 ? Q : XYZZ<Fq>::inf();
    for (int i = 0; i < l_log; ++i) Wt = Wt.dbl();
    Wt.add(T0);
    for (int i = 0; i < chunk_log; ++i) Wt = Wt.dbl();
    if (slots == 3) { for (int i = 0; i < 3; ++i) A = A.dbl(); U.add(A); }
    U.add(Wt);
    if (t == 0) U.add(Q);
    if (t < n) sh[t] = U;
    __syncthreads();
    lds_tree_reduce<Fq>(sh, n, t, COMBINE_THREADS, [] { __syncthreads(); });
    if (t == 0) store_norm_dev(out + 24 * ((size_t)w * gridDim.y + set), sh[0]);
}
__global__ __launch_bounds__(64) void k_msm_store_inf(uint32_t *out, uint32_t count) {
    const uint32_t i = blockIdx.x * blockDim.x + threadIdx.x;
    if (i < count) store_norm_dev(out + 24 * (size_t)i, XYZZ<Fq>::inf());
}
__global__ __launch_bounds__(256) void k_jac_to_records(const uint32_t *jac, size_t count, XYZZ<Fq> *rec) {
    const size_t i = (size_t)blockIdx.x * blockDim.x + threadIdx.x;
    if (i >= count) return;
    Fq X, Y, Z;
    for (int k = 0; k < 8; ++k) { X.v[k] = jac[24 * i + k]; Y.v[k] = jac[24 * i + 8 + k]; Z.v[k] = jac[24 * i + 16 + k]; }
    rec[i] = Z.is_zero() ? XYZZ<Fq>::inf() : XYZZ<Fq>{X, Y, Fq::one(), Fq::one()};
}
static size_t combine_lds_bytes(uint32_t cpw) { uint32_t n = 1; while (n < cpw && n < (uint32_t)COMBINE_THREADS) n <<= 1; return n * sizeof(LdsPoint<Fq>); }

static int sort_digits(MsmJob *job, const uint32_t *d_scalars, bool mont, const uint32_t *d_gather) {
    const MsmGeom g0 = job->g; const size_t n0 = job->n;
    if (job->merge > 1) { job->g.W /= job->merge; job->g.Wt = job->g.W; job->n *= job->merge; }
    if (job->multi > 1) { job->g.W *= job->multi; job->g.Wt = job->g.W; }
    const MsmGeom g = job->g; const size_t n = job->n;
    hipStream_t s = job->sort_stream ? job->sort_stream : job->stream;
    const size_t total = (size_t)g.W * g.B;
    uint32_t slice_len = (uint32_t)std::min<size_t>(65536, std::max<size_t>(4096, ((n + 15) / 16 + 1023) / 1024 * 1024));
    uint32_t S = (uint32_t)std::max<size_t>(1, (n + slice_len - 1) / slice_len);
    size_t nblk = (total + 1024 * SCAN_ITEMS - 1) / (1024 * SCAN_ITEMS);
    if (nblk > 1024) { set_error("msm: too many buckets for the block scan"); return ZKG_ERROR; }
    if (job->digits.reserve(std::max<size_t>(1, n * g.W) * 4) || job->hist.reserve((size_t)g.W * S * g.B * 4) || job->counts.reserve(total * 4) ||
        job->offsets.reserve((total + 1) * 4) || job->scan_sums.reserve(1024 * 4) || job->class_hist.reserve((HEAVY_T_MAX + 2) * 4) ||
        job->order.reserve(total * 4) || job->sorted.reserve(std::max<size_t>(1, n * g.W) * 4)) return ZKG_ERROR;
    uint32_t *digits = job->digits.as<uint32_t>(), *hist = job->hist.as<uint32_t>(), *counts = job->counts.as<uint32_t>(),
             *offsets = job->offsets.as<uint32_t>(), *sums = job->scan_sums.as<uint32_t>(), *chist = job->class_hist.as<uint32_t>();
    uint32_t cbits = 6;
    static const uint32_t bin_avg = getenv("ZKG_RX_AVG") ? (uint32_t)atoi(getenv("ZKG_RX_AVG")) : RX_BIN_AVG;
    while (cbits < RX_MAX_CBITS && cbits + 1 < g.c - 1 && (n >> cbits) > bin_avg) ++cbits;
    const bool two_pass = !job->one_pass_sort && g.c >= 12 && n >= 49152 && (n >> cbits) <= RX_FINE_MAX && n <= ((size_t)1 << (31 - (g.c - 1 - cbits)));
    {
        ZeroList zl{};
        int k = 0;
        zl.p[k] = chist; zl.words[k++] = HEAVY_T_MAX + 2;
        for (MsmGroup &gr : job->group) if (gr.nsets) {
            if (gr.heavy_counters.reserve(8 * MSM_MAX_SETS)) return ZKG_ERROR;
            zl.p[k] = gr.heavy_counters.as<uint32_t>(); zl.words[k++] = 2 * MSM_MAX_SETS;
        }
        if (two_pass) {
            const uint32_t nbins = g.W << cbits;
            if (job->rx_meta.reserve((3 * (size_t)nbins + 8) * 4)) return ZKG_ERROR;
            zl.p[k] = job->rx_meta.as<uint32_t>(); zl.words[k++] = 3 * nbins + 8;
        }
        const dim3 dg((unsigned)((n0 + 255) / 256));
        const bool four = !d_gather && (n0 & 3) == 0 && g0.w0 == 0 && g0.ws == 1 && g0.W == g0.Wt;
        const dim3 dg4((unsigned)((n0 / 4 + 255) / 256));
        if (job->multi > 1) {
            const dim3 dgm(dg.x, job->multi);
            if (g0.c == 16) hipLaunchKernelGGL(k_digits_multi<16>, dgm, dim3(256), 0, s, d_scalars, job->multi_stride, n0, (int)mont, job->merge, digits, zl);
            else if (g0.c == 12) hipLaunchKernelGGL(k_digits_multi<12>, dgm, dim3(256), 0, s, d_scalars, job->multi_stride, n0, (int)mont, job->merge, digits, zl);
            else hipLaunchKernelGGL(k_digits_multi_any, dgm, dim3(256), 0, s, d_scalars, job->multi_stride, n0, (int)mont, g0, job->merge, digits, zl);
        }
        else if (four && g0.c == 16) hipLaunchKernelGGL(k_digits_c4<16>, dg4, dim3(256), 0, s, d_scalars, n0, (int)mont, g0, digits, zl);
        else if (four && g0.c == 12) hipLaunchKernelGGL(k_digits_c4<12>, dg4, dim3(256), 0, s, d_scalars, n0, (int)mont, g0, digits, zl);
        else if (g0.c == 16) hipLaunchKernelGGL(k_digits_c<16>, dg, dim3(256), 0, s, d_scalars, d_gather, n0, (int)mont, g0, digits, zl);
        else if (g0.c == 12) hipLaunchKernelGGL(k_digits_c<12>, dg, dim3(256), 0, s, d_scalars, d_gather, n0, (int)mont, g0, digits, zl);
        else hipLaunchKernelGGL(k_digits, dg, dim3(256), 0, s, d_scalars, d_gather, n0, (int)mont, g0, digits, zl);
    }
    if (two_pass) {
        const uint32_t fbits = g.c - 1 - cbits, CB = 1u << cbits, nbins = g.W * CB, S1 = (uint32_t)((n + RX_SLICE - 1) / RX_SLICE);
        if (job->rx_tmp.reserve(n * g.W * 4) || job->rx_meta.reserve((3 * (size_t)nbins + 8) * 4)) return ZKG_ERROR;
        uint32_t *cnt = job->rx_meta.as<uint32_t>(), *base = cnt + nbins, *cursor = base + nbins + 1, *tmp = job->rx_tmp.as<uint32_t>();
        hipLaunchKernelGGL(k_rx_count, dim3(S1, g.W), dim3(1024), 0, s, digits, n, fbits, cbits, cnt);
        hipLaunchKernelGGL(k_rx_scan, dim3(1), dim3(1024), 0, s, cnt, nbins, base, cursor, offsets + total);
        static const int wg_env = getenv("ZKG_SORT_WG") ? atoi(getenv("ZKG_SORT_WG")) : 0;
        const bool half = (wg_env ? wg_env == 512 : job->sort_stream != nullptr) && fbits <= 9;
        if (half) {
            const uint32_t S2 = (uint32_t)((n + 512 * RX_PER_THREAD - 1) / (512 * RX_PER_THREAD));
            hipLaunchKernelGGL(k_rx_scatter<512>, dim3(S2, g.W), dim3(512), (512 * RX_PER_THREAD + 4 * RX_MAX_CB + 8) * 4, s, digits, n, fbits, cbits, base, cursor, tmp);
            hipLaunchKernelGGL(k_rx_fine<512>, dim3(CB, g.W), dim3(512), (RX_FINE_MAX + 3 * (1u << fbits)) * 4, s, tmp, fbits, cbits, g.B, base, counts, offsets,
                               job->sorted.as<uint32_t>());
        } else {
            hipLaunchKernelGGL(k_rx_scatter<1024>, dim3(S1, g.W), dim3(1024), (RX_SLICE + 4 * RX_MAX_CB + 8) * 4, s, digits, n, fbits, cbits, base, cursor, tmp);
            hipLaunchKernelGGL(k_rx_fine<1024>, dim3(CB, g.W), dim3(1024), (RX_FINE_MAX + 3 * (1u << fbits)) * 4, s, tmp, fbits, cbits, g.B, base, counts, offsets,
                               job->sorted.as<uint32_t>());
        }
    } else {
    hipLaunchKernelGGL(k_hist, dim3(S, g.W), dim3(SORT_THREADS), g.B * 4, s, digits, n, g.B, S, slice_len, hist);
    hipLaunchKernelGGL(k_colscan, dim3((unsigned)((total + 255) / 256)), dim3(256), 0, s, hist, g.B, S, total, counts);
    hipLaunchKernelGGL(k_scan_blocks, dim3((unsigned)nblk), dim3(1024), 0, s, counts, offsets, sums, total);
    hipLaunchKernelGGL(k_scan_sums, dim3(1), dim3(1024), 0, s, sums, (uint32_t)nblk, offsets + total);
    hipLaunchKernelGGL(k_scan_apply, dim3((unsigned)nblk), dim3(1024), 0, s, offsets, sums, total);
    hipLaunchKernelGGL(k_place, dim3(S, g.W), dim3(SORT_THREADS), g.B * 4, s, digits, n, g.B, S, slice_len, hist, offsets, job->sorted.as<uint32_t>());
    }
    hipLaunchKernelGGL(k_class_hist, dim3((unsigned)((total + 1023) / 1024)), dim3(1024), 0, s, counts, offsets, total, chist);
    hipLaunchKernelGGL(k_class_scan, dim3(1), dim3(1024), 0, s, chist, offsets, total);
    hipLaunchKernelGGL(k_order_place, dim3((unsigned)((total + 1023) / 1024)), dim3(1024), 0, s, counts, offsets, total, chist, job->order.as<uint32_t>());
    if (hipGetLastError() != hipSuccess) { set_error("msm sort launch failed"); return ZKG_ERROR; }
    return ZKG_OK;
}

MsmJob *msm_job_create(hipStream_t s, bool own_stream, bool high_priority) {
    MsmJob *j = new MsmJob();
    j->stream = s;
    if (own_stream) {
        int prio_lo = 0, prio_hi = 0;
        (void)hipDeviceGetStreamPriorityRange(&prio_lo, &prio_hi);
        if (!hip_ok(hipStreamCreateWithPriority(&j->stream, hipStreamNonBlocking, high_priority ? prio_hi : prio_lo), "hipStreamCreate", __FILE__, __LINE__)) { delete j; return nullptr; }
        j->own_stream = true;
    }
    return j;
}
void msm_job_set_window(MsmJob *j, int c) { if (j) j->window_hint = c; }
bool crit_priority_enabled() { static const bool on = !(getenv("ZKG_CRIT_PRIO") && atoi(getenv("ZKG_CRIT_PRIO")) == 0); return on; }
void msm_job_set_critical(MsmJob *j, bool critical) { if (j) j->critical = critical && crit_priority_enabled(); }
void msm_job_set_row_merge(MsmJob *j, uint32_t f) { if (j) j->merge_hint = f ? f : 1; }
void msm_job_set_skewed(MsmJob *j, bool skewed) { if (j) j->one_pass_sort = skewed; }
void msm_job_set_window_subset(MsmJob *j, uint32_t w0, uint32_t ws) { if (j) { j->w0 = w0; j->ws = ws ? ws : 1; } }
hipStream_t msm_job_stream(MsmJob *j) { return j->stream; }
void msm_job_destroy(MsmJob *j) {
    if (!j) return;
    for (DevBuf *b : {&j->digits, &j->hist, &j->counts, &j->offsets, &j->scan_sums, &j->class_hist, &j->order, &j->sorted, &j->rx_tmp, &j->rx_meta}) b->release();
    for (auto &gr : j->group) gr.release();
    if (j->aux) { (void)hipStreamSynchronize(j->aux); (void)hipStreamDestroy(j->aux); }
    if (j->ev_fork) (void)hipEventDestroy(j->ev_fork);
    if (j->ev_join) (void)hipEventDestroy(j->ev_join);
    if (j->own_stream) (void)hipStreamDestroy(j->stream);
    delete j;
}

static MsmJob g_default_job;
static MsmJob g_piece_job;
static hipStream_t g_sort_hi = nullptr;

int msm_job_launch(MsmJob *job, const MsmBases *sets, int nsets, const uint32_t *d_scalars, size_t n, bool scalars_mont, const uint32_t *d_gather) {
    static const bool dbg = getenv("ZKG_DEBUG_TIMING") != nullptr;
    auto t0 = std::chrono::steady_clock::now();
    auto lap = [&](const char *w) { if (dbg) fprintf(stderr, "[zkg]     %-18s %8.3f ms\n", w, std::chrono::duration<float, std::milli>(std::chrono::steady_clock::now() - t0).count()); };
    if (n >= ((size_t)1 << 31) || nsets < 0 || nsets > MSM_MAX_SETS) { set_error("msm: bad size"); return ZKG_ERROR; }
    bool any_table = false;
    for (int i = 0; i < nsets; ++i) any_table = any_table || sets[i].level_stride != 0;
    for (int i = 0; i < nsets; ++i) if ((sets[i].level_stride != 0) != any_table) { set_error("msm: table and plain base sets cannot share a launch"); return ZKG_ERROR; }
    if (any_table && (job->w0 != 0 || job->ws != 1 || job->window_hint <= 0)) { set_error("msm: a table launch covers all windows at the table's window size"); return ZKG_ERROR; }
    job->g = pick_geom(n, job->window_hint, job->w0, job->ws); job->n = n;
    job->empty = false; job->multi = 1;
    MsmBases by_field[2][MSM_MAX_SETS];
    for (MsmGroup &gr : job->group) gr.nsets = 0;
    job->group[0].g2 = false; job->group[1].g2 = true;
    for (int i = 0; i < nsets; ++i) { MsmGroup &gr = job->group[sets[i].g2 ? 1 : 0]; by_field[sets[i].g2 ? 1 : 0][gr.nsets] = sets[i]; gr.out_index[gr.nsets] = gr.nsets; ++gr.nsets; }
    if (job->g.W == 0 || n == 0) { job->empty = true; return ZKG_OK; }
    if ((uint64_t)n * job->g.W >= ((uint64_t)1 << 32)) { set_error("msm: n * windows exceeds the 32-bit index space of the sorted list (n < 2^28)"); return ZKG_ERROR; }
    job->merge = 1;
    if (any_table && job->merge_hint > 1 && !d_gather && job->g.W % job->merge_hint == 0 && (uint64_t)n * job->merge_hint < ((uint64_t)1 << 31)) {
        bool ok = true;
        for (int i = 0; i < nsets; ++i) ok = ok && sets[i].level_stride == n && sets[i].index_sub == 0 && !sets[i].remap;
        if (ok) job->merge = job->merge_hint;
    }
    job->converted_aside = false;
    {
        MsmGroup &g1 = job->group[0];
        if (!any_table && !d_gather && g1.nsets == 1 && by_field[0][0].index_sub == 0 && !by_field[0][0].remap && !by_field[0][0].p29) {
            if (!job->aux && (hipStreamCreateWithFlags(&job->aux, hipStreamNonBlocking) != hipSuccess || hipEventCreateWithFlags(&job->ev_fork, hipEventDisableTiming) != hipSuccess ||
                              hipEventCreateWithFlags(&job->ev_join, hipEventDisableTiming) != hipSuccess)) { set_error("msm: side stream"); return ZKG_ERROR; }
            if (g1.bases29.reserve(n * sizeof(Rec64))) return ZKG_ERROR;
            ZK_HIP(hipEventRecord(job->ev_fork, job->stream));
            ZK_HIP(hipStreamWaitEvent(job->aux, job->ev_fork, 0));
            hipLaunchKernelGGL(k_bases_to29, dim3((unsigned)((n + 255) / 256)), dim3(256), 0, job->aux, reinterpret_cast<const Affine<Fq> *>(by_field[0][0].p), n, g1.bases29.as<Rec64>());
            ZK_HIP(hipEventRecord(job->ev_join, job->aux));
            job->converted_aside = true;
        }
    }
    auto fail = [&] { if (job->converted_aside) { (void)hipStreamSynchronize(job->aux); job->converted_aside = false; } return ZKG_ERROR; };
    if (sort_digits(job, d_scalars, scalars_mont, d_gather)) return fail();
    if (job->sort_stream && job->sort_stream != job->stream) {
        if (hipEventRecord(job->ev_sorted, job->sort_stream) != hipSuccess || hipStreamWaitEvent(job->stream, job->ev_sorted, 0) != hipSuccess) return fail();
    }
    if (job->merge > 1) {
        for (int k = 0; k < 2; ++k) for (int i = 0; i < job->group[k].nsets; ++i) by_field[k][i].level_stride *= job->merge;
    }
    lap("sort enqueued");
    const bool timed_field_g2 = job->group[0].nsets == 0;
    if (job->group[1].nsets && launch_accumulate<Fq2>(job, job->group[1], by_field[1], d_gather, job == &g_default_job && timed_field_g2)) return fail();
    if (job->group[0].nsets && launch_accumulate<Fq>(job, job->group[0], by_field[0], d_gather, job == &g_default_job || job == &g_piece_job)) return fail();
    lap("accum enqueued");
    return ZKG_OK;
}
bool msm_multi_supported(size_t n, int c, uint32_t count) {
    const MsmGeom g = pick_geom(n, c);
    return c > 0 && count >= 1 && n >= 1 && (uint64_t)n * g.W * count < ((uint64_t)1 << 31) &&
           ((uint64_t)g.W * g.B * count + 1024 * SCAN_ITEMS - 1) / (1024 * SCAN_ITEMS) <= 1024;
}
int msm_job_launch_multi(MsmJob *job, const MsmBases *sets, int nsets, const uint32_t *d_scalars, size_t n, size_t scalar_stride, uint32_t count, bool scalars_mont) {
    bool ok = job->w0 == 0 && job->ws == 1 && nsets >= 1 && nsets <= MSM_MAX_SETS && msm_multi_supported(n, job->window_hint, count);
    for (int i = 0; i < nsets && ok; ++i) ok = sets[i].level_stride != 0 && !sets[i].remap && sets[i].index_sub == 0;
    if (!ok) { set_error("msm: unsupported multi launch"); return ZKG_ERROR; }
    job->g = pick_geom(n, job->window_hint); job->n = n;
    job->empty = false; job->converted_aside = false;
    MsmBases by_field[2][MSM_MAX_SETS];
    for (MsmGroup &gr : job->group) gr.nsets = 0;
    job->group[0].g2 = false; job->group[1].g2 = true;
    for (int i = 0; i < nsets; ++i) { MsmGroup &gr = job->group[sets[i].g2 ? 1 : 0]; by_field[sets[i].g2 ? 1 : 0][gr.nsets] = sets[i]; gr.out_index[gr.nsets] = gr.nsets; ++gr.nsets; }
    job->merge = 1;
    if (job->merge_hint > 1 && job->g.W % job->merge_hint == 0) {
        bool m = true;
        for (int i = 0; i < nsets; ++i) m = m && sets[i].level_stride == n;
        if (m) job->merge = job->merge_hint;
    }
    job->multi = count; job->multi_stride = scalar_stride;
    if (sort_digits(job, d_scalars, scalars_mont, nullptr)) return ZKG_ERROR;
    for (int k = 0; k < 2; ++k) for (int i = 0; i < job->group[k].nsets; ++i) by_field[k][i].level_stride *= job->merge;
    if (job->group[1].nsets && launch_accumulate<Fq2>(job, job->group[1], by_field[1], nullptr, false)) return ZKG_ERROR;
    if (job->group[0].nsets && launch_accumulate<Fq>(job, job->group[0], by_field[0], nullptr, false)) return ZKG_ERROR;
    return ZKG_OK;
}
int msm_job_finish_multi(MsmJob *job, G1 *out_g1, G2 *out_g2) {
    ZK_HIP(hipStreamSynchronize(job->stream));
    const int n1 = job->group[0].nsets, n2 = job->group[1].nsets;
    host_parallel_for((int)job->multi, [&](int p) {
        for (int k = 0; k < n1; ++k) out_g1[p * n1 + k] = host_combine<Fq>(job, job->group[0], k, p);
        for (int k = 0; k < n2; ++k) out_g2[p * n2 + k] = host_combine<Fq2>(job, job->group[1], k, p);
    });
    return ZKG_OK;
}
int msm_job_finish(MsmJob *job, G1 *out_g1, G2 *out_g2) {
    static const bool dbg = getenv("ZKG_DEBUG_TIMING") != nullptr;
    const auto t0 = std::chrono::steady_clock::now();
    ZK_HIP(hipStreamSynchronize(job->stream));
    const auto t1 = std::chrono::steady_clock::now();
    struct Lap { bool on; std::chrono::steady_clock::time_point a, b; ~Lap() { if (on) fprintf(stderr, "[zkg]     job finish: waited %.3f ms, host combine %.3f ms\n", std::chrono::duration<float, std::milli>(b - a).count(), std::chrono::duration<float, std::milli>(std::chrono::steady_clock::now() - b).count()); } } lap_{dbg, t0, t1};
    for (int k = 0; k < job->group[0].nsets; ++k) out_g1[k] = job->empty ? G1::inf() : host_combine<Fq>(job, job->group[0], k);
    for (int k = 0; k < job->group[1].nsets; ++k) out_g2[k] = job->empty ? G2::inf() : host_combine<Fq2>(job, job->group[1], k);
    return ZKG_OK;
}

void msm_job_set_device_finish(MsmJob *j, bool on) { if (j) j->dev_finish = on; }
int msm_job_finish_dev(MsmJob *job, uint64_t *d_out) {
    const MsmGroup &gr = job->group[0];
    if (!job->dev_finish || job->group[1].nsets || gr.nsets < 1) { set_error("msm_job_finish_dev: a device-finish launch of G1 sets only"); return ZKG_ERROR; }
    const uint32_t vectors = job->multi > 1 ? job->multi : 1;
    uint32_t *out = reinterpret_cast<uint32_t *>(d_out);
    if (job->empty) {
        const uint32_t count = vectors * (uint32_t)gr.nsets;
        hipLaunchKernelGGL(k_msm_store_inf, dim3((count + 63) / 64), dim3(64), 0, job->stream, out, count);
    } else {
        if (!gr.table || gr.red_windows != vectors) { set_error("msm_job_finish_dev: table sets only (a plain set's windows need the Horner doublings)"); return ZKG_ERROR; }
        hipLaunchKernelGGL(k_msm_combine, dim3(vectors, (unsigned)gr.nsets), dim3(COMBINE_THREADS), combine_lds_bytes(gr.cpw), job->stream,
                           gr.red_out.as<XYZZ<Fq>>(), gr.cpw, gr.red_slots, gr.chunk_log, gr.red_stride, out);
    }
    if (hipGetLastError() != hipSuccess) { set_error("msm combine launch failed"); return ZKG_ERROR; }
    return ZKG_OK;
}
int msm_combine_records(const uint64_t *records_jac, size_t cpw, int slots, int chunk_log, size_t vectors, uint64_t *out_jac) {
    if (!records_jac || !out_jac || cpw < 1 || cpw > ((size_t)1 << 16) || (slots != 2 && slots != 3) || chunk_log < 0 || chunk_log > 24 || vectors < 1 || vectors > 1024) {
        set_error("zkg_msm_combine_gpu: bad argument (1 <= cpw <= 2^16, slots 2 or 3, 0 <= chunk_log <= 24, 1 <= vectors <= 1024)"); return ZKG_ERROR;
    }
    const size_t count = vectors * cpw * (size_t)slots;
    ScopedDevBuf in, rec, out;
    if (in.reserve(count * 96) || rec.reserve(count * sizeof(XYZZ<Fq>)) || out.reserve(vectors * 96)) return ZKG_ERROR;
    ZK_HIP(hipMemcpy(in.p, records_jac, count * 96, hipMemcpyHostToDevice));
    hipLaunchKernelGGL(k_jac_to_records, dim3((unsigned)((count + 255) / 256)), dim3(256), 0, nullptr, in.as<uint32_t>(), count, rec.as<XYZZ<Fq>>());
    hipLaunchKernelGGL(k_msm_combine, dim3((unsigned)vectors, 1), dim3(COMBINE_THREADS), combine_lds_bytes((uint32_t)cpw), nullptr,
                       rec.as<XYZZ<Fq>>(), (uint32_t)cpw, slots, chunk_log, (size_t)0, out.as<uint32_t>());
    if (hipGetLastError() != hipSuccess) { set_error("msm combine launch failed"); return ZKG_ERROR; }
    ZK_HIP(hipMemcpy(out_jac, out.p, vectors * 96, hipMemcpyDeviceToHost));
    return ZKG_OK;
}


int msm_shared(const G1Affine *const *d_g1_bases, int n_g1, const G2Affine *d_g2_bases, const uint32_t *d_scalars, size_t n,
               bool scalars_mont, G1 *out_g1, G2 *out_g2, hipStream_t s, uint32_t w0, uint32_t ws, bool mostly_bits) {
    if (n_g1 < 0 || n_g1 + (d_g2_bases ? 1 : 0) > MSM_MAX_SETS) { set_error("msm: too many base sets"); return ZKG_ERROR; }
    std::lock_guard<std::mutex> lk(g_default_job.mu);
    g_dominant_timer.new_call();
    g_default_job.stream = s; g_default_job.w0 = w0; g_default_job.ws = ws ? ws : 1; g_default_job.one_pass_sort = mostly_bits;
    MsmBases sets[MSM_MAX_SETS]; int nsets = 0;
    for (int i = 0; i < n_g1; ++i) { sets[nsets] = MsmBases(); sets[nsets].p = d_g1_bases[i]; ++nsets; }
    if (d_g2_bases) { sets[nsets] = MsmBases(); sets[nsets].p = d_g2_bases; sets[nsets].g2 = true; ++nsets; }
    if (n >= ((size_t)1 << 28)) { set_error("msm: at most 2^28 - 1 points per call"); return ZKG_ERROR; }
    const size_t PIECE = (size_t)1 << 23;
    if (n <= PIECE || w0 != 0 || g_default_job.ws != 1) {
        if (msm_job_launch(&g_default_job, sets, nsets, d_scalars, n, scalars_mont, nullptr)) return ZKG_ERROR;
        return msm_job_finish(&g_default_job, out_g1, out_g2);
    }
    G1 acc1[MSM_MAX_SETS]; G2 acc2[MSM_MAX_SETS];
    for (int i = 0; i < MSM_MAX_SETS; ++i) { acc1[i] = G1::inf(); acc2[i] = G2::inf(); }
    for (size_t lo = 0; lo < n; lo += PIECE) {
        const size_t cnt = std::min(PIECE, n - lo);
        MsmBases piece[MSM_MAX_SETS];
        for (int i = 0; i < nsets; ++i) { piece[i] = sets[i]; piece[i].p = (const char *)sets[i].p + lo * (sets[i].g2 ? sizeof(G2Affine) : sizeof(G1Affine)); }
        G1 p1[MSM_MAX_SETS]; G2 p2[MSM_MAX_SETS];
        if (msm_job_launch(&g_default_job, piece, nsets, d_scalars + 8 * lo, cnt, scalars_mont, nullptr) || msm_job_finish(&g_default_job, p1, p2)) return ZKG_ERROR;
        for (int i = 0; i < n_g1; ++i) acc1[i].add(p1[i]);
        if (d_g2_bases) acc2[0].add(p2[0]);
    }
    for (int i = 0; i < n_g1; ++i) out_g1[i] = acc1[i];
    if (d_g2_bases) out_g2[0] = acc2[0];
    return ZKG_OK;
}

int msm_g1_host_scalars(const G1Affine *d_bases, const uint32_t *h_scalars, size_t n, bool mont, G1 *out, hipStream_t s) {
    if (n >= ((size_t)1 << 28)) { set_error("msm: at most 2^28 - 1 points per call"); return ZKG_ERROR; }
    if (!n) { *out = G1::inf(); return ZKG_OK; }
    static const int max_pieces = getenv("ZKG_MSM_PIECES") ? std::max(1, std::min(8, atoi(getenv("ZKG_MSM_PIECES")))) : 4;
    const bool pieces = max_pieces > 1 && n >= ((size_t)1 << 19) && n <= ((size_t)1 << 23);
    if (n > ((size_t)1 << 23)) {
        ScopedDevBuf tmp;
        if (tmp.reserve(n * 32)) return ZKG_ERROR;
        ZK_HIP(hipMemcpyAsync(tmp.p, h_scalars, n * 32, hipMemcpyHostToDevice, s));
        return msm_g1(d_bases, tmp.as<uint32_t>(), n, mont, out, s, false);
    }
    MsmJob &J = g_default_job;
    std::lock_guard<std::mutex> lk(J.mu);
    g_dominant_timer.new_call();
    if (J.hs_scalars.reserve(n * 32)) return ZKG_ERROR;
    if (!J.copy) {
        if (hipStreamCreateWithFlags(&J.copy, hipStreamNonBlocking) != hipSuccess) { J.copy = nullptr; set_error("msm: copy stream"); return ZKG_ERROR; }
        for (auto &e : J.ev_piece) if (hipEventCreateWithFlags(&e, hipEventDisableTiming) != hipSuccess) { set_error("msm: event"); return ZKG_ERROR; }
    }
    uint32_t *d_sc = J.hs_scalars.as<uint32_t>();
    J.stream = s; J.w0 = 0; J.ws = 1; J.one_pass_sort = false;
    MsmBases set; set.p = d_bases;
    if (!pieces) {
        ZK_HIP(hipMemcpyAsync(d_sc, h_scalars, n * 32, hipMemcpyHostToDevice, s));
        if (msm_job_launch(&J, &set, 1, d_sc, n, mont, nullptr)) return ZKG_ERROR;
        return msm_job_finish(&J, out, nullptr);
    }
    size_t cut[9]; int P = max_pieces;
    cut[P] = n;
    for (int k = P - 1; k >= 1; --k) cut[k] = (cut[k + 1] / 2) & ~(size_t)255;
    cut[0] = 0;
    if (const char *e = getenv("ZKG_MSM_CUTS")) {
        int k = 1; const char *q = e;
        while (*q && k < 8) { const long v = strtol(q, const_cast<char **>(&q), 10); if (v <= 0 || v >= 64) break; cut[k++] = (n * (size_t)v / 64) & ~(size_t)255; if (*q == ',') ++q; }
        if (k > 1) { P = k; cut[P] = n; for (int i = 1; i < P; ++i) if (cut[i] < cut[i - 1]) cut[i] = cut[i - 1]; }
    }
    for (int k = 0; k < P; ++k) {
        ZK_HIP(hipMemcpyAsync(d_sc + 8 * cut[k], h_scalars + 8 * cut[k], (cut[k + 1] - cut[k]) * 32, hipMemcpyHostToDevice, J.copy));
        ZK_HIP(hipEventRecord(J.ev_piece[k], J.copy));
    }
    MsmJob &K = g_piece_job;
    if (!g_sort_hi) {
        int lo = 0, hi = 0; (void)hipDeviceGetStreamPriorityRange(&lo, &hi);
        bool ok = hipStreamCreateWithPriority(&g_sort_hi, hipStreamNonBlocking, hi) == hipSuccess;
        for (MsmJob *w : {&J, &K}) ok = ok && hipEventCreateWithFlags(&w->ev_sorted, hipEventDisableTiming) == hipSuccess && hipEventCreateWithFlags(&w->ev_acc_done, hipEventDisableTiming) == hipSuccess;
        if (!ok) { g_sort_hi = nullptr; set_error("msm: sort stream"); return ZKG_ERROR; }
    }
    hipStream_t s_hi = g_sort_hi;
    if (!J.aux && (hipStreamCreateWithFlags(&J.aux, hipStreamNonBlocking) != hipSuccess || hipEventCreateWithFlags(&J.ev_fork, hipEventDisableTiming) != hipSuccess ||
                   hipEventCreateWithFlags(&J.ev_join, hipEventDisableTiming) != hipSuccess)) { set_error("msm: side stream"); return ZKG_ERROR; }
    if (J.group[0].bases29.reserve(n * sizeof(Rec64))) return ZKG_ERROR;
    ZK_HIP(hipEventRecord(J.ev_fork, s));
    ZK_HIP(hipStreamWaitEvent(J.aux, J.ev_fork, 0));
    hipLaunchKernelGGL(k_bases_to29, dim3((unsigned)((n + 255) / 256)), dim3(256), 0, J.aux, reinterpret_cast<const Affine<Fq> *>(d_bases), n, J.group[0].bases29.as<Rec64>());
    ZK_HIP(hipEventRecord(J.ev_join, J.aux));
    ZK_HIP(hipStreamWaitEvent(s, J.ev_join, 0));
    ZK_HIP(hipStreamWaitEvent(s_hi, J.ev_fork, 0));
    const int c = (int)pick_geom(n, J.window_hint).c;
    const int saved_hint = J.window_hint, saved_hint_k = K.window_hint;
    J.window_hint = c; K.window_hint = c; K.bucket_owner = &J; K.w0 = 0; K.ws = 1; K.one_pass_sort = false; K.stream = s;
    int rc = ZKG_OK; bool started = false; bool used[2] = {false, false};
    for (int k = 0; k < P && rc == ZKG_OK; ++k) {
        if (cut[k + 1] == cut[k] && k + 1 < P) continue;
        const int which = (P - 1 - k) & 1;
        MsmJob &W = which ? K : J;
        MsmBases piece = set; piece.p = reinterpret_cast<const char *>(d_bases) + cut[k] * sizeof(G1Affine);
        piece.p29 = J.group[0].bases29.as<Rec64>() + cut[k];
        W.resume = started; W.defer_reduce = k + 1 < P; started = true;
        W.sort_stream = s_hi;
        if (hipStreamWaitEvent(s_hi, J.ev_piece[k], 0) != hipSuccess) { rc = ZKG_ERROR; break; }
        if (used[which] && hipStreamWaitEvent(s_hi, W.ev_acc_done, 0) != hipSuccess) { rc = ZKG_ERROR; break; }
        rc = msm_job_launch(&W, &piece, 1, d_sc + 8 * cut[k], cut[k + 1] - cut[k], mont, nullptr);
        if (rc == ZKG_OK && hipEventRecord(W.ev_acc_done, s) != hipSuccess) rc = ZKG_ERROR;
        used[which] = true;
    }
    J.resume = false; J.defer_reduce = false; J.window_hint = saved_hint; J.sort_stream = nullptr;
    K.resume = false; K.defer_reduce = false; K.window_hint = saved_hint_k; K.bucket_owner = nullptr; K.sort_stream = nullptr; K.stream = nullptr;
    if (rc != ZKG_OK) { (void)hipStreamSynchronize(J.copy); (void)hipStreamSynchronize(s_hi); (void)hipStreamSynchronize(s); return ZKG_ERROR; }
    return msm_job_finish(&J, out, nullptr);
}

int msm_g1(const G1Affine *d_bases, const uint32_t *d_scalars, size_t n, bool mont, G1 *out, hipStream_t s, bool mostly_bits) {
    return msm_shared(&d_bases, 1, nullptr, d_scalars, n, mont, out, nullptr, s, 0, 1, mostly_bits);
}
int msm_g2(const G2Affine *d_bases, const uint32_t *d_scalars, size_t n, bool mont, G2 *out, hipStream_t s, bool mostly_bits) {
    return msm_shared(nullptr, 0, d_bases, d_scalars, n, mont, nullptr, out, s, 0, 1, mostly_bits);
}

template <class F>
static int window_table_build_t(WindowTable &t, const Affine<F> *d_bases, size_t n, int c, hipStream_t s) {
    t.n = n; t.c = c; t.W = (SCALAR_BITS + c - 1) / c; t.g2 = sizeof(F) != sizeof(Fq);
    if (t.buf.reserve(std::max<size_t>(1, n) * t.W * sizeof(Affine<F>))) return ZKG_ERROR;
    if (!n) return ZKG_OK;
    Affine<F> *lv = t.buf.as<Affine<F>>();
    ZK_HIP(hipMemcpyAsync(lv, d_bases, n * sizeof(Affine<F>), hipMemcpyDeviceToDevice, s));
    constexpr int K = sizeof(F) != sizeof(Fq) ? 2 : 4;
    for (int w = 1; w < t.W; w += K)
        hipLaunchKernelGGL((k_table_levels<F, K>), dim3((unsigned)((n + 255) / 256)), dim3(256), 0, s, lv + (size_t)(w - 1) * n, lv + (size_t)w * n, n, (uint32_t)c,
                           std::min(K, t.W - w));
    if (hipGetLastError() != hipSuccess) { set_error("window table launch failed"); return ZKG_ERROR; }
    return ZKG_OK;
}
int window_table_build_g1(WindowTable &t, const G1Affine *d_bases, size_t n, int c, hipStream_t s) { return window_table_build_t<Fq>(t, d_bases, n, c, s); }
int window_table_records29(WindowTable &t, hipStream_t s) {
    if (t.g2) { set_error("window_table_records29: G1 tables only"); return ZKG_ERROR; }
    const size_t total = t.n * (size_t)t.W;
    if (t.rec29.reserve(std::max<size_t>(1, total) * sizeof(Rec64))) return ZKG_ERROR;
    if (total) hipLaunchKernelGGL(k_bases_to29, dim3((unsigned)((total + 255) / 256)), dim3(256), 0, s, t.buf.as<Affine<Fq>>(), total, t.rec29.as<Rec64>());
    if (hipGetLastError() != hipSuccess) { set_error("window table records launch failed"); return ZKG_ERROR; }
    return ZKG_OK;
}
int window_table_build_g2(WindowTable &t, const G2Affine *d_bases, size_t n, int c, hipStream_t s) { return window_table_build_t<Fq2>(t, d_bases, n, c, s); }

int witness_classify(const Fr *d_z, size_t n1, uint8_t *d_tags, uint32_t *d_listed, uint32_t *d_count, hipStream_t s, const uint32_t *d_subset_pos) {
    ZK_HIP(hipMemsetAsync(d_count, 0, 8, s));
    if (n1) hipLaunchKernelGGL(k_classify, dim3((unsigned)((n1 + 255) / 256)), dim3(256), 0, s, d_z, n1, d_tags, d_listed, d_count, d_subset_pos);
    return hipGetLastError() == hipSuccess ? ZKG_OK : ZKG_ERROR;
}
template <class F> static int gather_points_t(const Affine<F> *d_src, const uint32_t *d_idx, size_t count, uint32_t index_sub, Affine<F> *d_out, hipStream_t s) {
    if (count) hipLaunchKernelGGL(k_gather_points<F>, dim3((unsigned)((count + 255) / 256)), dim3(256), 0, s, d_src, d_idx, count, index_sub, d_out);
    return hipGetLastError() == hipSuccess ? ZKG_OK : ZKG_ERROR;
}
int gather_points_g1(const G1Affine *d_src, const uint32_t *d_idx, size_t count, uint32_t index_sub, G1Affine *d_out, hipStream_t s) { return gather_points_t<Fq>(d_src, d_idx, count, index_sub, d_out, s); }
int gather_points_g2(const G2Affine *d_src, const uint32_t *d_idx, size_t count, uint32_t index_sub, G2Affine *d_out, hipStream_t s) { return gather_points_t<Fq2>(d_src, d_idx, count, index_sub, d_out, s); }
template <class F> static int scatter_points_t(const Affine<F> *d_src, const uint32_t *d_idx, size_t count, Affine<F> *d_out, hipStream_t s) {
    if (count) hipLaunchKernelGGL(k_scatter_points<F>, dim3((unsigned)((count + 255) / 256)), dim3(256), 0, s, d_src, d_idx, count, d_out);
    return hipGetLastError() == hipSuccess ? ZKG_OK : ZKG_ERROR;
}
int scatter_points_g1(const G1Affine *d_src, const uint32_t *d_idx, size_t count, G1Affine *d_out, hipStream_t s) { return scatter_points_t<Fq>(d_src, d_idx, count, d_out, s); }
int scatter_points_g2(const G2Affine *d_src, const uint32_t *d_idx, size_t count, G2Affine *d_out, hipStream_t s) { return scatter_points_t<Fq2>(d_src, d_idx, count, d_out, s); }
template <class F>
static int ones_sum_launch_t(OnesSum &o, const MsmBases *sets, int nsets, const uint8_t *d_tags, size_t n1, hipStream_t s, size_t tag_stride = 0, uint32_t vecs = 1) {
    if (nsets < 1 || nsets > MSM_MAX_SETS) { set_error("ones-sum: bad set count"); return ZKG_ERROR; }
    const uint32_t span = (uint32_t)std::min<size_t>(8192, std::max<size_t>(1024, ((n1 + 255) / 256 + 255) / 256 * 256));
    const unsigned blocks = (unsigned)std::max<size_t>(1, (n1 + span - 1) / span);
    o.g2 = sizeof(F) != sizeof(Fq); o.nsets = nsets;
    const size_t vec_stride = (size_t)nsets * (blocks + 1), host_bytes = std::max<size_t>(MSM_MAX_SETS, (size_t)vecs * nsets) * sizeof(G2);
    if (o.partials.reserve(vecs * vec_stride * sizeof(XYZZ<F>))) return ZKG_ERROR;
    if (o.host_bytes < host_bytes) {
        if (o.host) (void)hipHostFree(o.host);
        o.host = nullptr; o.host_bytes = 0;
        if (!hip_ok(hipHostMalloc(&o.host, host_bytes, hipHostMallocDefault), "hipHostMalloc", __FILE__, __LINE__)) return ZKG_ERROR;
        o.host_bytes = host_bytes;
    }
    XYZZ<F> *part = o.partials.as<XYZZ<F>>();
    ViewSet<F> views;
    for (int i = 0; i < MSM_MAX_SETS; ++i) { const MsmBases &b = sets[i < nsets ? i : 0]; views.v[i] = BaseView<F>{reinterpret_cast<const Affine<F> *>(b.p), 0, nullptr, b.index_sub, 1, nullptr}; }
    hipLaunchKernelGGL(k_ones_sum<F>, dim3(blocks, (unsigned)nsets, vecs), dim3(256), 256 * sizeof(LdsPoint<F>) + (size_t)span * 4, s, views, d_tags, n1, span, part, tag_stride, vec_stride);
    hipLaunchKernelGGL(k_sum_partials<F>, dim3((unsigned)nsets, vecs), dim3(256), 256 * sizeof(LdsPoint<F>), s, part, blocks, vec_stride);
    if (hipGetLastError() != hipSuccess) { set_error("ones-sum launch failed"); return ZKG_ERROR; }
    if (vecs > 1) {
        ZK_HIP(hipMemcpy2DAsync(o.host, sizeof(XYZZ<F>), part + blocks, (blocks + 1) * sizeof(XYZZ<F>), sizeof(XYZZ<F>), (size_t)vecs * nsets, hipMemcpyDeviceToHost, s));
        return ZKG_OK;
    }
    for (int i = 0; i < nsets; ++i)
        ZK_HIP(hipMemcpyAsync((char *)o.host + (size_t)i * sizeof(XYZZ<F>), part + (size_t)i * (blocks + 1) + blocks, sizeof(XYZZ<F>), hipMemcpyDeviceToHost, s));
    return ZKG_OK;
}
int ones_sum_launch(OnesSum &o, const MsmBases *sets, int nsets, const uint8_t *d_tags, size_t n1, hipStream_t s) {
    for (int i = 1; i < nsets; ++i) if (sets[i].g2 != sets[0].g2) { set_error("ones-sum: one field per launch"); return ZKG_ERROR; }
    return sets[0].g2 ? ones_sum_launch_t<Fq2>(o, sets, nsets, d_tags, n1, s) : ones_sum_launch_t<Fq>(o, sets, nsets, d_tags, n1, s);
}
int ones_sum_launch_multi(OnesSum &o, const MsmBases *sets, int nsets, const uint8_t *d_tags, size_t tag_stride, size_t n1, uint32_t count, hipStream_t s) {
    for (int i = 1; i < nsets; ++i) if (sets[i].g2 != sets[0].g2) { set_error("ones-sum: one field per launch"); return ZKG_ERROR; }
    if (count < 1 || count > 65535) { set_error("ones-sum: bad witness count"); return ZKG_ERROR; }
    return sets[0].g2 ? ones_sum_launch_t<Fq2>(o, sets, nsets, d_tags, n1, s, tag_stride, count) : ones_sum_launch_t<Fq>(o, sets, nsets, d_tags, n1, s, tag_stride, count);
}
void OnesSum::release() { partials.release(); if (host) (void)hipHostFree(host); host = nullptr; host_bytes = 0; }

static constexpr int FB_WINDOWS = 32, FB_DIGITS = 255, FB_K = 4;
template <class F>
__global__ __launch_bounds__(256) void k_fixed_table(const Affine<F> *rows , Affine<F> *table) {
    const uint32_t t = blockIdx.x * blockDim.x + threadIdx.x;
    if (t >= FB_WINDOWS * FB_DIGITS) return;
    const uint32_t j = t / FB_DIGITS, d = t % FB_DIGITS + 1;
    const Affine<F> r = rows[j];
    XYZZ<F> acc = XYZZ<F>::inf();
    for (int bit = 7; bit >= 0; --bit) { acc = acc.dbl(); if ((d >> bit) & 1u) acc.madd(r); }
    XYZZ<F> fin = acc;
    table[t] = fin.to_affine().normalized();
}
template <class F>
__global__ __launch_bounds__(256) void k_fixed_base(const Affine<F> *table, const uint32_t *scalars, size_t n, int mont, Affine<F> *out) {
    const size_t lane = (size_t)blockIdx.x * blockDim.x + threadIdx.x, i0 = lane * FB_K;
    if (i0 >= n) return;
    F x[FB_K], y[FB_K], zz[FB_K], zzz[FB_K];
#pragma unroll
    for (int k = 0; k < FB_K; ++k) {
        XYZZ<F> acc = XYZZ<F>::inf();
        if (i0 + k < n) {
            Fr f;
            for (int j = 0; j < 8; ++j) f.v[j] = scalars[8 * (i0 + k) + j];
            if (mont) f = f.from_mont();
            else f = f.normalized();
            for (int j = 0; j < FB_WINDOWS; ++j) {
                const uint32_t d = (f.v[j >> 2] >> (8 * (j & 3))) & 255u;
                if (d) acc.madd(table[j * FB_DIGITS + d - 1]);
            }
        }
        x[k] = acc.x; y[k] = acc.y; zz[k] = acc.zz; zzz[k] = acc.zzz;
    }
    F pre[FB_K], run = F::one();
#pragma unroll
    for (int k = 0; k < FB_K; ++k) { pre[k] = run; if (!zzz[k].is_zero()) run = run * zzz[k]; }
    F inv = inverse_fast(run);
#pragma unroll
    for (int k = FB_K - 1; k >= 0; --k) {
        if (i0 + k >= n) continue;
        if (zzz[k].is_zero()) { out[i0 + k] = Affine<F>::inf(); continue; }
        F zi = inv * pre[k];
        inv = inv * zzz[k];
        F t = zi * zz[k];
        F zi2 = t.sqr();
        out[i0 + k] = Affine<F>{x[k] * zi2, y[k] * zi}.normalized();
    }
}

template <class F> struct FixedTableCache { std::mutex mu; std::vector<std::pair<Affine<F>, DevBuf>> entries; };
template <class F> static FixedTableCache<F> &fixed_cache() { static FixedTableCache<F> c; return c; }
template <class F>
static const Affine<F> *fixed_table_for(const Affine<F> &base, hipStream_t s) {
    FixedTableCache<F> &c = fixed_cache<F>();
    std::lock_guard<std::mutex> lk(c.mu);
    for (auto &e : c.entries) if (memcmp(&e.first, &base, sizeof(base)) == 0) return e.second.template as<Affine<F>>();
    std::vector<Affine<F>> rows(FB_WINDOWS);
    XYZZ<F> cur = XYZZ<F>::from_affine(base);
    for (int j = 0; j < FB_WINDOWS; ++j) { rows[j] = cur.to_affine(); for (int k = 0; k < 8; ++k) cur = cur.dbl(); }
    DevBuf d_rows, d_table;
    if (d_rows.reserve(rows.size() * sizeof(Affine<F>)) || d_table.reserve((size_t)FB_WINDOWS * FB_DIGITS * sizeof(Affine<F>))) return nullptr;
    if (!hip_ok(hipMemcpyAsync(d_rows.p, rows.data(), rows.size() * sizeof(Affine<F>), hipMemcpyHostToDevice, s), "H2D", __FILE__, __LINE__)) return nullptr;
    hipLaunchKernelGGL(k_fixed_table<F>, dim3((FB_WINDOWS * FB_DIGITS + 255) / 256), dim3(256), 0, s, d_rows.as<Affine<F>>(), d_table.as<Affine<F>>());
    const bool ok = hipGetLastError() == hipSuccess && hip_ok(hipStreamSynchronize(s), "sync", __FILE__, __LINE__);
    d_rows.release();
    if (!ok) { d_table.release(); set_error("fixed-base table build failed"); return nullptr; }
    c.entries.emplace_back(base, d_table);
    return c.entries.back().second.template as<Affine<F>>();
}
template <class F>
static int fixed_base(const Affine<F> &base, const uint32_t *d_scalars, size_t n, Affine<F> *d_out, hipStream_t s, bool mont) {
    const Affine<F> *table = fixed_table_for<F>(base, s);
    if (!table) return ZKG_ERROR;
    const size_t lanes = (n + FB_K - 1) / FB_K;
    if (n) hipLaunchKernelGGL(k_fixed_base<F>, dim3((unsigned)((lanes + 255) / 256)), dim3(256), 0, s, table, d_scalars, n, (int)mont, d_out);
    hipError_t e = hipGetLastError();
    ZK_HIP(hipStreamSynchronize(s));
    if (e != hipSuccess) { set_error("fixed_base launch failed"); return ZKG_ERROR; }
    return ZKG_OK;
}
int fixed_base_g1(const G1Affine &base, const uint32_t *d_scalars, size_t n, G1Affine *d_out, hipStream_t s, bool mont) { return fixed_base<Fq>(base, d_scalars, n, d_out, s, mont); }
int fixed_base_g2(const G2Affine &base, const uint32_t *d_scalars, size_t n, G2Affine *d_out, hipStream_t s, bool mont) { return fixed_base<Fq2>(base, d_scalars, n, d_out, s, mont); }
static void fixed_tables_release() {
    { auto &c = fixed_cache<Fq>(); std::lock_guard<std::mutex> lk(c.mu); for (auto &e : c.entries) e.second.release(); c.entries.clear(); }
    { auto &c = fixed_cache<Fq2>(); std::lock_guard<std::mutex> lk(c.mu); for (auto &e : c.entries) e.second.release(); c.entries.clear(); }
}

int msm_configure() {
    bool ok = hipFuncSetAttribute((const void *)k_bucket_reduce<Fq2, RED_L_LOG_SMALL>, hipFuncAttributeMaxDynamicSharedMemorySize, 2 * RedGeom<Fq2>::LANES * (int)sizeof(LdsPoint<Fq2>)) == hipSuccess;
    ok = ok && hipFuncSetAttribute((const void *)k_bucket_reduce<Fq2, RED_L_LOG_TINY>, hipFuncAttributeMaxDynamicSharedMemorySize, 2 * RedGeom<Fq2>::LANES * (int)sizeof(LdsPoint<Fq2>)) == hipSuccess;
    ok = ok && hipFuncSetAttribute((const void *)k_bucket_reduce<Fq2, RED_L_LOG_LARGE>, hipFuncAttributeMaxDynamicSharedMemorySize, 2 * RedGeom<Fq2>::LANES * (int)sizeof(LdsPoint<Fq2>)) == hipSuccess;
    ok = ok && hipFuncSetAttribute((const void *)k_heavy_parts<Fq2>, hipFuncAttributeMaxDynamicSharedMemorySize, 256 * (int)sizeof(LdsPoint<Fq2>)) == hipSuccess;
    ok = ok && hipFuncSetAttribute((const void *)k_heavy_merge<Fq2>, hipFuncAttributeMaxDynamicSharedMemorySize, 256 * (int)sizeof(LdsPoint<Fq2>)) == hipSuccess;
    ok = ok && hipFuncSetAttribute((const void *)k_bucket_fold<Fq2>, hipFuncAttributeMaxDynamicSharedMemorySize, (int)FOLD_THREADS * (int)sizeof(LdsPoint<Fq2>)) == hipSuccess;
    ok = ok && hipFuncSetAttribute((const void *)k_ones_sum<Fq2>, hipFuncAttributeMaxDynamicSharedMemorySize, 256 * (int)sizeof(LdsPoint<Fq2>) + 8192 * 4) == hipSuccess;
    ok = ok && hipFuncSetAttribute((const void *)k_ones_sum<Fq>, hipFuncAttributeMaxDynamicSharedMemorySize, 256 * (int)sizeof(LdsPoint<Fq>) + 8192 * 4) == hipSuccess;
    ok = ok && hipFuncSetAttribute((const void *)k_sum_partials<Fq2>, hipFuncAttributeMaxDynamicSharedMemorySize, 256 * (int)sizeof(LdsPoint<Fq2>)) == hipSuccess;
    ok = ok && hipFuncSetAttribute((const void *)k_hist, hipFuncAttributeMaxDynamicSharedMemorySize, (1 << (MAX_C - 1)) * 4) == hipSuccess;
    ok = ok && hipFuncSetAttribute((const void *)k_place, hipFuncAttributeMaxDynamicSharedMemorySize, (1 << (MAX_C - 1)) * 4) == hipSuccess;
    ok = ok && hipFuncSetAttribute((const void *)k_bucket_reduce29l, hipFuncAttributeMaxDynamicSharedMemorySize, 4 * RedGeom<Fq>::LANES * (int)sizeof(LdsPoint29)) == hipSuccess;
    ok = ok && hipFuncSetAttribute((const void *)k_rx_scatter<1024>, hipFuncAttributeMaxDynamicSharedMemorySize, (RX_SLICE + 4 * RX_MAX_CB + 8) * 4) == hipSuccess;
    ok = ok && hipFuncSetAttribute((const void *)k_rx_scatter<512>, hipFuncAttributeMaxDynamicSharedMemorySize, (512 * RX_PER_THREAD + 4 * RX_MAX_CB + 8) * 4) == hipSuccess;
    ok = ok && hipFuncSetAttribute((const void *)k_rx_fine<1024>, hipFuncAttributeMaxDynamicSharedMemorySize, (RX_FINE_MAX + 3 * 1024) * 4) == hipSuccess;
    ok = ok && hipFuncSetAttribute((const void *)k_rx_fine<512>, hipFuncAttributeMaxDynamicSharedMemorySize, (RX_FINE_MAX + 3 * 1024) * 4) == hipSuccess;
    return ok ? ZKG_OK : ZKG_ERROR;
}
void msm_release_all() {
    fixed_tables_release();
    MsmJob &j = g_default_job;
    std::lock_guard<std::mutex> lk(j.mu);
    for (DevBuf *b : {&j.digits, &j.hist, &j.counts, &j.offsets, &j.scan_sums, &j.class_hist, &j.order, &j.sorted, &j.rx_tmp, &j.rx_meta}) b->release();
    for (auto &gr : j.group) gr.release();
    if (j.aux) { (void)hipStreamSynchronize(j.aux); (void)hipStreamDestroy(j.aux); j.aux = nullptr; }
    j.hs_scalars.release();
    {
        MsmJob &k = g_piece_job;
        if (g_sort_hi) { (void)hipStreamSynchronize(g_sort_hi); (void)hipStreamDestroy(g_sort_hi); g_sort_hi = nullptr; }
        for (DevBuf *b : {&k.digits, &k.hist, &k.counts, &k.offsets, &k.scan_sums, &k.class_hist, &k.order, &k.sorted, &k.rx_tmp, &k.rx_meta}) b->release();
        for (auto &gr : k.group) gr.release();
        if (k.aux) { (void)hipStreamSynchronize(k.aux); (void)hipStreamDestroy(k.aux); k.aux = nullptr; }
        if (k.ev_fork) { (void)hipEventDestroy(k.ev_fork); k.ev_fork = nullptr; }
        if (k.ev_join) { (void)hipEventDestroy(k.ev_join); k.ev_join = nullptr; }
        for (MsmJob *w : {&j, &k}) {
            if (w->ev_sorted) { (void)hipEventDestroy(w->ev_sorted); w->ev_sorted = nullptr; }
            if (w->ev_acc_done) { (void)hipEventDestroy(w->ev_acc_done); w->ev_acc_done = nullptr; }
        }
        k.stream = nullptr;
    }
    if (j.copy) { (void)hipStreamSynchronize(j.copy); (void)hipStreamDestroy(j.copy); j.copy = nullptr; }
    for (auto &e : j.ev_piece) if (e) { (void)hipEventDestroy(e); e = nullptr; }
    if (j.ev_fork) { (void)hipEventDestroy(j.ev_fork); j.ev_fork = nullptr; }
    if (j.ev_join) { (void)hipEventDestroy(j.ev_join); j.ev_join = nullptr; }
}

}
```

Baseline: 54.22.

## Fuse radix-sort scan into scatter/fine kernels and speed host window doubling

The separate k_rx_scan and k_class_scan kernels are removed. Bin base offsets are now computed on the fly from per-window totals and bin counts inside the scatter and fine kernels, and the class histogram is built inside k_rx_fine using several replicated copies to reduce atomic contention. On the host, repeated XYZZ doublings for window combination are replaced with a Jacobian doubling loop that uses a dedicated 64-bit Montgomery squaring routine. The device-to-host copy of reduction output also appears to change. Every block now performs redundant prefix sums, and k_order_place has to merge the histogram copies.

```diff
diff --git a/zklaim_amd/csrc/host/horner_jac.hpp b/zklaim_amd/csrc/host/horner_jac.hpp
--- /dev/null
+++ b/zklaim_amd/csrc/host/horner_jac.hpp
@@ -0,0 +1,66 @@
+#pragma once
+#include "../curve.hip.hpp"
+#include <cstring>
+
+namespace zk {
+
+static inline Fq fq_sqr_host(const Fq &a) {
+    typedef unsigned __int128 u128;
+    constexpr uint64_t P4[4] = {Fq::p64(0), Fq::p64(1), Fq::p64(2), Fq::p64(3)};
+    uint64_t A[4], r[8];
+    memcpy(A, a.v, 32);
+    u128 x = (u128)A[0] * A[1];                r[1] = (uint64_t)x; uint64_t c = (uint64_t)(x >> 64);
+    x = (u128)A[0] * A[2] + c;                 r[2] = (uint64_t)x; c = (uint64_t)(x >> 64);
+    x = (u128)A[0] * A[3] + c;                 r[3] = (uint64_t)x; r[4] = (uint64_t)(x >> 64);
+    x = (u128)A[1] * A[2] + r[3];              r[3] = (uint64_t)x; c = (uint64_t)(x >> 64);
+    x = (u128)A[1] * A[3] + r[4] + c;          r[4] = (uint64_t)x; r[5] = (uint64_t)(x >> 64);
+    x = (u128)A[2] * A[3] + r[5];              r[5] = (uint64_t)x; r[6] = (uint64_t)(x >> 64);
+    r[7] = r[6] >> 63;
+    for (int j = 6; j >= 2; --j) r[j] = (r[j] << 1) | (r[j - 1] >> 63);
+    r[1] <<= 1;
+    x = (u128)A[0] * A[0];                     r[0] = (uint64_t)x; c = (uint64_t)(x >> 64);
+    x = (u128)r[1] + c;                        r[1] = (uint64_t)x; c = (uint64_t)(x >> 64);
+    x = (u128)A[1] * A[1] + r[2] + c;          r[2] = (uint64_t)x; c = (uint64_t)(x >> 64);
+    x = (u128)r[3] + c;                        r[3] = (uint64_t)x; c = (uint64_t)(x >> 64);
+    x = (u128)A[2] * A[2] + r[4] + c;          r[4] = (uint64_t)x; c = (uint64_t)(x >> 64);
+    x = (u128)r[5] + c;                        r[5] = (uint64_t)x; c = (uint64_t)(x >> 64);
+    x = (u128)A[3] * A[3] + r[6] + c;          r[6] = (uint64_t)x; c = (uint64_t)(x >> 64);
+    r[7] += c;
+    uint64_t top = 0;
+    for (int i = 0; i < 4; ++i) {
+        const uint64_t m = r[i] * FqParams::INV64;
+        c = 0;
+        for (int j = 0; j < 4; ++j) { x = (u128)m * P4[j] + r[i + j] + c; r[i + j] = (uint64_t)x; c = (uint64_t)(x >> 64); }
+        x = (u128)r[i + 4] + c + top; r[i + 4] = (uint64_t)x; top = (uint64_t)(x >> 64);
+    }
+    uint64_t s[4]; unsigned long long br = 0;
+    for (int j = 0; j < 4; ++j) s[j] = __builtin_subcll(r[4 + j], P4[j], br, &br);
+    const uint64_t keep = 0ull - (uint64_t)br;
+    for (int j = 0; j < 4; ++j) s[j] ^= (s[j] ^ r[4 + j]) & keep;
+    Fq out; memcpy(out.v, s, 32);
+    return out;
+}
+
+template <class F> static inline XYZZ<F> xyzz_times_pow2(const XYZZ<F> &p, uint32_t n) {
+    if (p.is_inf() || n == 0) return p;
+    if constexpr (std::is_same<F, Fq>::value) {
+        if (n >= 3) {
+            Fq X = p.x * p.zz, Y = p.y * p.zzz, Z = p.zz;
+            for (uint32_t i = 0; i < n; ++i) {
+                const Fq A = fq_sqr_host(X), B = fq_sqr_host(Y), C = fq_sqr_host(B);
+                const Fq D = (fq_sqr_host(X + B) - A - C).dbl(), E = A.dbl() + A, E2 = fq_sqr_host(E);
+                Z = (Y * Z).dbl();
+                X = E2 - D.dbl();
+                Y = E * (D - X) - C.dbl().dbl().dbl();
+            }
+            if (Z.is_zero()) return XYZZ<Fq>::inf();
+            const Fq zz = fq_sqr_host(Z);
+            return {X, Y, zz, zz * Z};
+        }
+    }
+    XYZZ<F> r = p;
+    for (uint32_t i = 0; i < n; ++i) r = r.dbl();
+    return r;
+}
+
+}
diff --git a/zklaim_amd/csrc/msm.hip b/zklaim_amd/csrc/msm.hip
--- a/zklaim_amd/csrc/msm.hip
+++ b/zklaim_amd/csrc/msm.hip
@@ -1,5 +1,6 @@
 #include "common.hpp"
 #include "fq29.hip.hpp"
+#include "host/horner_jac.hpp"
 #include "../../include/zkg.h"
 #include <algorithm>
 #include <chrono>
@@ -20,6 +21,7 @@
 static constexpr int MAX_C = 16;
 static constexpr uint32_t HEAVY_S = 512;
 static constexpr uint32_t HEAVY_T_MAX = 1024;
+static constexpr uint32_t CLASS_HIST_COPIES = 8;
 static constexpr int HEAVY_PART_BLOCKS = 512, HEAVY_MERGE_BLOCKS = 128;
 static constexpr int SORT_THREADS = 1024;
 static constexpr int SCAN_ITEMS = 4;
@@ -291,11 +293,26 @@
 
 
 static constexpr uint32_t RX_MAX_CBITS = 10, RX_MAX_CB = 1u << RX_MAX_CBITS, RX_SLICE = 16384, RX_PER_THREAD = 16, RX_FINE_MAX = 8192, RX_BIN_AVG = 4096;
-__global__ __launch_bounds__(1024) void k_rx_count(const uint32_t *digits, size_t n, uint32_t fbits, uint32_t cbits, uint32_t *cnt) {
+ZK_D uint32_t heavy_threshold_dev(const uint32_t *offsets, size_t total_buckets, uint32_t divisor) {
+    uint32_t entries = offsets[total_buckets];
+    uint32_t avg6 = (uint32_t)(6 * (uint64_t)entries / total_buckets), slack = 8 + avg6 > 32 ? 32 : 8 + avg6;
+    uint32_t t = (uint32_t)(4 * (uint64_t)entries / total_buckets) + slack;
+    t = t > HEAVY_T_MAX ? HEAVY_T_MAX : t;
+    t /= divisor;
+    return t < 4 ? 4 : t;
+}
+ZK_D uint32_t wave_sum(uint32_t v) {
+#pragma unroll
+    for (int d = 32; d >= 1; d >>= 1) v += __shfl_xor(v, d, 64);
+    return v;
+}
+__global__ __launch_bounds__(1024) void k_rx_count(const uint32_t *digits, size_t n, uint32_t fbits, uint32_t cbits, uint32_t *cnt, uint32_t *wtot) {
     sort_wave_priority();
     __shared__ uint32_t c[RX_MAX_CB];
+    __shared__ uint32_t tot;
     const uint32_t sl = blockIdx.x, w = blockIdx.y, t = threadIdx.x, CB = 1u << cbits;
     if (t < CB) c[t] = 0;
+    if (t == 0) tot = 0;
     __syncthreads();
     size_t lo = (size_t)sl * RX_SLICE, hi = lo + RX_SLICE < n ? lo + RX_SLICE : n;
     const uint32_t *d = digits + (size_t)w * n;
@@ -310,37 +327,45 @@
     } else
     for (size_t i = lo + t; i < hi; i += 1024) { uint32_t code = d[i]; if (code) atomicAdd(&c[((code >> 1) - 1) >> fbits], 1u); }
     __syncthreads();
-    if (t < CB && c[t]) atomicAdd(&cnt[w * CB + t], c[t]);
-}
-__global__ __launch_bounds__(1024) void k_rx_scan(const uint32_t *cnt, uint32_t nbins, uint32_t *base, uint32_t *cursor, uint32_t *grand_total) {
-    sort_wave_priority();
-    __shared__ uint32_t part[1024];
-    const uint32_t t = threadIdx.x, per = (nbins + 1023) / 1024, lo = t * per, hi = lo + per < nbins ? lo + per : nbins;
-    uint32_t sum = 0;
-    for (uint32_t i = lo; i < hi; ++i) sum += cnt[i];
-    part[t] = sum;
-    __syncthreads();
-    for (uint32_t d = 1; d < 1024; d <<= 1) {
-        uint32_t x = (t >= d) ? part[t - d] : 0;
-        __syncthreads();
-        part[t] += x;
-        __syncthreads();
-    }
-    uint32_t run = part[t] - sum;
-    for (uint32_t i = lo; i < hi; ++i) { base[i] = run; cursor[i] = 0; run += cnt[i]; }
-    if (t == 1023) { base[nbins] = part[1023]; *grand_total = part[1023]; }
+    if (t < CB) {
+        const uint32_t mine = c[t];
+        if (mine) atomicAdd(&cnt[w * CB + t], mine);
+        const uint32_t in_wave = wave_sum(mine);
+        if ((t & 63) == 0 && in_wave) atomicAdd(&tot, in_wave);
+    }
+    __syncthreads();
+    if (t == 0 && tot) atomicAdd(&wtot[w], tot);
+}
+ZK_D uint32_t rx_entries_before(const uint32_t *cnt, const uint32_t *wtot, uint32_t w, uint32_t cb, uint32_t cbits) {
+    uint32_t v = 0;
+    for (uint32_t i = threadIdx.x; i < w; i += blockDim.x) v += wtot[i];
+    for (uint32_t b = threadIdx.x; b < cb; b += blockDim.x) v += cnt[(w << cbits) + b];
+    return v;
 }
 template <int T>
-__global__ __launch_bounds__(T) void k_rx_scatter(const uint32_t *digits, size_t n, uint32_t fbits, uint32_t cbits, const uint32_t *base, uint32_t *cursor,
-                                                   uint32_t *tmp) {
+__global__ __launch_bounds__(T) void k_rx_scatter(const uint32_t *digits, size_t n, uint32_t fbits, uint32_t cbits, const uint32_t *cnt, const uint32_t *wtot, uint32_t W,
+                                                   uint32_t *cursor, uint32_t *tmp, uint32_t *grand_total) {
     sort_wave_priority();
     extern __shared__ uint32_t lds_u32[];
     constexpr uint32_t SLICE = RX_PER_THREAD * T;
     const uint32_t CB = 1u << cbits;
-    uint32_t *stage = lds_u32, *c = lds_u32 + SLICE, *off = c + RX_MAX_CB, *gb = off + RX_MAX_CB + 1, *cur = gb + RX_MAX_CB;
+    uint32_t *stage = lds_u32, *c = lds_u32 + SLICE, *off = c + RX_MAX_CB, *gb = off + RX_MAX_CB + 1, *cur = gb + RX_MAX_CB, *wsum = cur + RX_MAX_CB;
     const uint32_t sl = blockIdx.x, w = blockIdx.y, t = threadIdx.x;
     for (uint32_t b = t; b < CB; b += T) c[b] = 0;
-    __syncthreads();
+    if (t < 2) wsum[t] = 0;
+    __syncthreads();
+    const uint32_t b0 = t, b1 = t + T;
+    const uint32_t g0 = b0 < CB ? cnt[w * CB + b0] : 0, g1 = b1 < CB ? cnt[w * CB + b1] : 0;
+    {
+        const uint32_t below = wave_sum(rx_entries_before(cnt, wtot, w, 0, cbits));
+        if ((t & 63) == 0 && below) atomicAdd(&wsum[0], below);
+        if (sl == 0 && w == 0) {
+            uint32_t all = 0;
+            for (uint32_t i = t; i < W; i += T) all += wtot[i];
+            all = wave_sum(all);
+            if ((t & 63) == 0 && all) atomicAdd(&wsum[1], all);
+        }
+    }
     size_t lo = (size_t)sl * SLICE, hi = lo + SLICE < n ? lo + SLICE : n;
     const uint32_t *d = digits + (size_t)w * n;
     uint32_t code[RX_PER_THREAD];
@@ -361,20 +386,23 @@
 #pragma unroll
     for (uint32_t j = 0; j < RX_PER_THREAD; ++j) if (code[j]) atomicAdd(&c[((code[j] >> 1) - 1) >> fbits], 1u);
     __syncthreads();
-    const uint32_t b0 = t, b1 = t + T;
-    if (b0 < CB) off[b0] = c[b0];
-    if (b1 < CB) off[b1] = c[b1];
+    if (b0 < CB) { off[b0] = c[b0]; gb[b0] = g0; }
+    if (b1 < CB) { off[b1] = c[b1]; gb[b1] = g1; }
     __syncthreads();
     for (uint32_t dd = 1; dd < CB; dd <<= 1) {
-        const uint32_t x0 = (b0 < CB && b0 >= dd) ? off[b0 - dd] : 0, x1 = (b1 < CB && b1 >= dd) ? off[b1 - dd] : 0;
-        __syncthreads();
-        if (b0 < CB) off[b0] += x0;
-        if (b1 < CB) off[b1] += x1;
+        const bool in0 = b0 < CB && b0 >= dd, in1 = b1 < CB && b1 >= dd;
+        const uint32_t x0 = in0 ? off[b0 - dd] : 0, x1 = in1 ? off[b1 - dd] : 0, y0 = in0 ? gb[b0 - dd] : 0, y1 = in1 ? gb[b1 - dd] : 0;
+        __syncthreads();
+        if (b0 < CB) { off[b0] += x0; gb[b0] += y0; }
+        if (b1 < CB) { off[b1] += x1; gb[b1] += y1; }
         __syncthreads();
     }
     if (t == 0) off[CB] = off[CB - 1];
-    __syncthreads();
-    for (uint32_t b = t; b < CB; b += T) { off[b] -= c[b]; gb[b] = c[b] ? base[w * CB + b] + atomicAdd(&cursor[w * CB + b], c[b]) : 0; cur[b] = 0; }
+    if (t == 0 && sl == 0 && w == 0) *grand_total = wsum[1];
+    __syncthreads();
+    const uint32_t wstart = wsum[0];
+    if (b0 < CB) { off[b0] -= c[b0]; gb[b0] = c[b0] ? wstart + (gb[b0] - g0) + atomicAdd(&cursor[w * CB + b0], c[b0]) : 0; cur[b0] = 0; }
+    if (b1 < CB) { off[b1] -= c[b1]; gb[b1] = c[b1] ? wstart + (gb[b1] - g1) + atomicAdd(&cursor[w * CB + b1], c[b1]) : 0; cur[b1] = 0; }
     __syncthreads();
     const uint32_t fmask = (1u << fbits) - 1;
 #pragma unroll
@@ -391,9 +419,10 @@
         for (uint32_t p = a + lane; p < b; p += 64) tmp[g + (p - a)] = stage[p];
     }
 }
-ZK_D void rx_fine_offsets(uint32_t *cf, uint32_t *of, uint32_t FB, uint32_t t, uint32_t start, size_t gb0, uint32_t *counts, uint32_t *offsets) {
+ZK_D void rx_fine_offsets(uint32_t *cf, uint32_t *of, uint32_t FB, uint32_t t, uint32_t start, size_t gb0, uint32_t *counts, uint32_t *offsets, uint32_t *h, uint32_t heavy_t,
+                          uint32_t *class_hist) {
     const uint32_t T = blockDim.x;
-    if (t < FB) of[t] = cf[t];
+    if (t < FB) { const uint32_t c = cf[t]; of[t] = c; atomicAdd(&h[c > heavy_t ? heavy_t + 1 : c], 1u); }
     __syncthreads();
     for (uint32_t d = 1; d < FB; d <<= 1) {
         uint32_t x = (t < FB && t >= d) ? of[t - d] : 0;
@@ -404,9 +433,11 @@
     if (t < FB) of[t] -= cf[t];
     __syncthreads();
     for (uint32_t f = t; f < FB; f += T) { counts[gb0 + f] = cf[f]; offsets[gb0 + f] = start + of[f]; }
+    uint32_t *copy = class_hist + ((blockIdx.x + blockIdx.y) % CLASS_HIST_COPIES) * (HEAVY_T_MAX + 2);
+    for (uint32_t i = t; i < heavy_t + 2; i += T) if (h[i]) atomicAdd(&copy[i], h[i]);
 }
 ZK_D void rx_fine_big_bin(const uint32_t *tmp, uint32_t fbits, uint32_t start, uint32_t cnt, size_t gb0, uint32_t *cf, uint32_t *of, uint32_t *cur, uint32_t *counts,
-                          uint32_t *offsets, uint32_t *sorted) {
+                          uint32_t *offsets, uint32_t *sorted, uint32_t *h, uint32_t heavy_t, uint32_t *class_hist) {
     const uint32_t FB = 1u << fbits, sh = 32 - fbits, low = (1u << sh) - 1, t = threadIdx.x, T = blockDim.x;
     const bool giant = cnt > 8 * RX_FINE_MAX;
     if (!giant) {
@@ -421,7 +452,7 @@
         }
     }
     __syncthreads();
-    rx_fine_offsets(cf, of, FB, t, start, gb0, counts, offsets);
+    rx_fine_offsets(cf, of, FB, t, start, gb0, counts, offsets, h, heavy_t, class_hist);
     if (!giant) {
         for (uint32_t p = t; p < cnt; p += T) { uint32_t e = tmp[start + p], f = e >> sh; sorted[start + of[f] + atomicAdd(&cur[f], 1u)] = e & low; }
         return;
@@ -439,18 +470,25 @@
     }
 }
 template <int T>
-__global__ __launch_bounds__(T) void k_rx_fine(const uint32_t *tmp, uint32_t fbits, uint32_t cbits, uint32_t B, const uint32_t *base, uint32_t *counts, uint32_t *offsets,
-                                                uint32_t *sorted) {
+__global__ __launch_bounds__(T) void k_rx_fine(const uint32_t *tmp, uint32_t fbits, uint32_t cbits, uint32_t B, const uint32_t *bin_cnt, const uint32_t *wtot, uint32_t *counts,
+                                                uint32_t *offsets, size_t total, uint32_t *class_hist, uint32_t *sorted) {
     sort_wave_priority();
     extern __shared__ uint32_t lds_u32[];
     const uint32_t FB = 1u << fbits, sh = 32 - fbits, low = (1u << sh) - 1;
-    uint32_t *bufB = lds_u32, *cf = bufB + RX_FINE_MAX, *of = cf + FB, *cur = of + FB;
+    uint32_t *bufB = lds_u32, *cf = bufB + RX_FINE_MAX, *of = cf + FB, *cur = of + FB, *h = bufB, *before = h + HEAVY_T_MAX + 2;
     const uint32_t cb = blockIdx.x, w = blockIdx.y, t = threadIdx.x, bin = (w << cbits) + cb;
-    const uint32_t start = base[bin], cnt = base[bin + 1] - start;
     const size_t gb0 = (size_t)w * B + (size_t)cb * FB;
     for (uint32_t f = t; f < FB; f += T) { cf[f] = 0; cur[f] = 0; }
-    __syncthreads();
-    if (cnt > RX_FINE_MAX) { rx_fine_big_bin(tmp, fbits, start, cnt, gb0, cf, of, cur, counts, offsets, sorted); return; }
+    for (uint32_t i = t; i < HEAVY_T_MAX + 2; i += T) h[i] = 0;
+    if (t == 0) { before[0] = 0; before[1] = heavy_threshold_dev(offsets, total, 1); }
+    __syncthreads();
+    {
+        const uint32_t v = wave_sum(rx_entries_before(bin_cnt, wtot, w, cb, cbits));
+        if ((t & 63) == 0 && v) atomicAdd(&before[0], v);
+    }
+    __syncthreads();
+    const uint32_t start = before[0], heavy_t = before[1], cnt = bin_cnt[bin];
+    if (cnt > RX_FINE_MAX) { rx_fine_big_bin(tmp, fbits, start, cnt, gb0, cf, of, cur, counts, offsets, sorted, h, heavy_t, class_hist); return; }
     uint32_t ent[RX_FINE_MAX / T];
 #pragma unroll
     for (uint32_t j = 0; j < RX_FINE_MAX / T; ++j) {
@@ -459,7 +497,8 @@
         if (p < cnt) atomicAdd(&cf[ent[j] >> sh], 1u);
     }
     __syncthreads();
-    rx_fine_offsets(cf, of, FB, t, start, gb0, counts, offsets);
+    rx_fine_offsets(cf, of, FB, t, start, gb0, counts, offsets, h, heavy_t, class_hist);
+    __syncthreads();
 #pragma unroll
     for (uint32_t j = 0; j < RX_FINE_MAX / T; ++j) {
         if (t + j * T >= cnt) continue;
@@ -468,15 +507,6 @@
     }
     __syncthreads();
     for (uint32_t p = t; p < cnt; p += T) sorted[start + p] = bufB[p];
-}
-
-ZK_D uint32_t heavy_threshold_dev(const uint32_t *offsets, size_t total_buckets, uint32_t divisor) {
-    uint32_t entries = offsets[total_buckets];
-    uint32_t avg6 = (uint32_t)(6 * (uint64_t)entries / total_buckets), slack = 8 + avg6 > 32 ? 32 : 8 + avg6;
-    uint32_t t = (uint32_t)(4 * (uint64_t)entries / total_buckets) + slack;
-    t = t > HEAVY_T_MAX ? HEAVY_T_MAX : t;
-    t /= divisor;
-    return t < 4 ? 4 : t;
 }
 
 __global__ __launch_bounds__(1024) void k_class_hist(const uint32_t *counts, const uint32_t *offsets, size_t total, uint32_t *class_hist) {
@@ -491,35 +521,38 @@
     __syncthreads();
     for (uint32_t i = t; i < nc; i += 1024) if (h[i]) atomicAdd(&class_hist[i], h[i]);
 }
-__global__ __launch_bounds__(1024) void k_class_scan(uint32_t *class_hist, const uint32_t *offsets, size_t total) {
+__global__ __launch_bounds__(1024) void k_order_place(const uint32_t *counts, const uint32_t *offsets, size_t total, const uint32_t *class_hist, uint32_t *class_cursor,
+                                                       uint32_t *order) {
     sort_wave_priority();
-    __shared__ uint32_t part[1024];
-    const uint32_t heavy_t = heavy_threshold_dev(offsets, total, 1), nc = heavy_t + 2, t = threadIdx.x;
-    uint32_t v0 = 2 * t < nc ? class_hist[nc - 1 - 2 * t] : 0, v1 = 2 * t + 1 < nc ? class_hist[nc - 2 - 2 * t] : 0;
-    part[t] = v0 + v1;
-    __syncthreads();
-    for (uint32_t d = 1; d < 1024; d <<= 1) {
-        uint32_t x = (t >= d) ? part[t - d] : 0;
-        __syncthreads();
-        part[t] += x;
-        __syncthreads();
-    }
-    const uint32_t before = part[t] - v0 - v1;
-    if (2 * t < nc) class_hist[nc - 1 - 2 * t] = before;
-    if (2 * t + 1 < nc) class_hist[nc - 2 - 2 * t] = before + v0;
-}
-__global__ __launch_bounds__(1024) void k_order_place(const uint32_t *counts, const uint32_t *offsets, size_t total, uint32_t *class_cursor, uint32_t *order) {
-    sort_wave_priority();
-    __shared__ uint32_t h[HEAVY_T_MAX + 2];
-    const uint32_t heavy_t = heavy_threshold_dev(offsets, total, 1);
-    const uint32_t t = threadIdx.x, nc = heavy_t + 2;
-    for (uint32_t i = t; i < nc; i += 1024) h[i] = 0;
-    __syncthreads();
+    __shared__ uint32_t h[HEAVY_T_MAX + 2], first[HEAVY_T_MAX + 2], wave_total[16], threshold;
+    const uint32_t t = threadIdx.x, wave = t >> 6, lane = t & 63;
+    for (uint32_t i = t; i < HEAVY_T_MAX + 2; i += 1024) h[i] = 0;
+    if (t == 0) threshold = heavy_threshold_dev(offsets, total, 1);
+    __syncthreads();
+    const uint32_t heavy_t = threshold, nc = heavy_t + 2;
     size_t gb = (size_t)blockIdx.x * 1024 + t;
     uint32_t cls = 0, rank = 0;
     if (gb < total) { uint32_t c = counts[gb]; cls = c > heavy_t ? heavy_t + 1 : c; rank = atomicAdd(&h[cls], 1u); }
-    __syncthreads();
-    for (uint32_t i = t; i < nc; i += 1024) if (h[i]) h[i] = atomicAdd(&class_cursor[i], h[i]);
+    uint32_t v0 = 0, v1 = 0, incl = 0;
+    if (128 * wave < nc) {
+        for (uint32_t k = 0; k < CLASS_HIST_COPIES; ++k) {
+            const uint32_t *copy = class_hist + k * (HEAVY_T_MAX + 2);
+            if (2 * t < nc) v0 += copy[nc - 1 - 2 * t];
+            if (2 * t + 1 < nc) v1 += copy[nc - 2 - 2 * t];
+        }
+        incl = v0 + v1;
+        for (uint32_t d = 1; d < 64; d <<= 1) { const uint32_t y = __shfl_up(incl, d, 64); if (lane >= d) incl += y; }
+    }
+    if (lane == 63) wave_total[wave] = incl;
+    __syncthreads();
+    if (128 * wave < nc) {
+        uint32_t before = incl - v0 - v1;
+        for (uint32_t k = 0; k < wave; ++k) before += wave_total[k];
+        if (2 * t < nc) first[nc - 1 - 2 * t] = before;
+        if (2 * t + 1 < nc) first[nc - 2 - 2 * t] = before + v0;
+    }
+    __syncthreads();
+    for (uint32_t i = t; i < nc; i += 1024) if (h[i]) h[i] = first[i] + atomicAdd(&class_cursor[i], h[i]);
     __syncthreads();
     if (gb < total) order[h[cls] + rank] = (uint32_t)gb;
 }
@@ -1177,7 +1210,7 @@
     SetLayout L; L.buckets = total_buckets; L.items = max_items; L.heavy = max_heavy; L.partials = max_items; L.folded = BP; L.red_out = gr.nred * 3;
     if (gr.heavy_items.reserve(ns * max_items * sizeof(HeavyItem)) || gr.heavy_buckets.reserve(ns * max_heavy * sizeof(HeavyBucket)) ||
         gr.heavy_counters.reserve(8 * MSM_MAX_SETS) || gr.heavy_partials.reserve(ns * max_items * sizeof(XYZZ<F>)) ||
-        bucket_buf.reserve(ns * total_buckets * std::max(sizeof(XYZZ<F>), sizeof(Bucket29))) || gr.red_out.reserve(ns * L.red_out * sizeof(XYZZ<F>)) || ((gr.red_stride = L.red_out), false) ||
+        bucket_buf.reserve(ns * total_buckets * std::max(sizeof(XYZZ<F>), sizeof(Bucket29))) || (job->dev_finish && gr.red_out.reserve(ns * L.red_out * sizeof(XYZZ<F>))) || ((gr.red_stride = L.red_out), false) ||
         (gr.table && gr.folded.reserve(ns * (size_t)BP * std::max(sizeof(XYZZ<F>), sizeof(Bucket29)))) || (!job->dev_finish && gr.host_reserve(ns * L.red_out * sizeof(XYZZ<F>)))) return ZKG_ERROR;
     XYZZ<F> *buckets = bucket_buf.as<XYZZ<F>>();
     ViewSet<F> views;
@@ -1234,6 +1267,7 @@
         return ZKG_OK;
     }
     const XYZZ<F> *red_in = buckets; size_t in_stride = L.buckets;
+    XYZZ<F> *red_dst = job->dev_finish ? gr.red_out.as<XYZZ<F>>() : reinterpret_cast<XYZZ<F> *>(gr.host_red);
     bool folded29 = false;
     if constexpr (sizeof(F) == sizeof(Fq)) {
         if (gr.table && out29) {
@@ -1251,7 +1285,7 @@
     }
     if constexpr (sizeof(F) == sizeof(Fq)) {
         const size_t lds = 2 * RG::LANES * sizeof(LdsPoint29);
-        const void *rin = red_in; XYZZ<Fq> *rout = reinterpret_cast<XYZZ<Fq> *>(gr.red_out.p);
+        const void *rin = red_in; XYZZ<Fq> *rout = reinterpret_cast<XYZZ<Fq> *>(red_dst);
         auto launch_red = [&](auto kern, unsigned threads) { hipLaunchKernelGGL(kern, dim3((unsigned)gr.nred, ns), dim3(threads), lds, s, rin, g.B, gr.cpw, rout, in_stride, L.red_out, job->critical ? 1 : 0); };
         if (out29 && red_l_log == RED_L_LOG_LARGE) {
             gr.red_slots = 3;
@@ -1268,17 +1302,15 @@
     } else {
         if (red_l_log == RED_L_LOG_LARGE)
             hipLaunchKernelGGL((k_bucket_reduce<F, RED_L_LOG_LARGE>), dim3((unsigned)gr.nred, ns), dim3(RG::THREADS), 2 * RG::LANES * sizeof(LdsPoint<F>), s,
-                               red_in, g.B, gr.cpw, gr.red_out.as<XYZZ<F>>(), in_stride, L.red_out);
+                               red_in, g.B, gr.cpw, red_dst, in_stride, L.red_out);
         else if (red_l_log == RED_L_LOG_SMALL)
             hipLaunchKernelGGL((k_bucket_reduce<F, RED_L_LOG_SMALL>), dim3((unsigned)gr.nred, ns), dim3(RG::THREADS), 2 * RG::LANES * sizeof(LdsPoint<F>), s,
-                               red_in, g.B, gr.cpw, gr.red_out.as<XYZZ<F>>(), in_stride, L.red_out);
+                               red_in, g.B, gr.cpw, red_dst, in_stride, L.red_out);
         else
             hipLaunchKernelGGL((k_bucket_reduce<F, RED_L_LOG_TINY>), dim3((unsigned)gr.nred, ns), dim3(RG::THREADS), 2 * RG::LANES * sizeof(LdsPoint<F>), s,
-                               red_in, g.B, gr.cpw, gr.red_out.as<XYZZ<F>>(), in_stride, L.red_out);
+                               red_in, g.B, gr.cpw, red_dst, in_stride, L.red_out);
     }
     if (hipGetLastError() != hipSuccess) { set_error("msm kernel launch failed"); return ZKG_ERROR; }
-    if (job->dev_finish) return ZKG_OK;
-    ZK_HIP(hipMemcpyAsync(gr.host_red, gr.red_out.p, ns * L.red_out * sizeof(XYZZ<F>), hipMemcpyDeviceToHost, s));
     return ZKG_OK;
 }
 
@@ -1298,8 +1330,8 @@
             if (ch >= 1) { suffix.add(P); weighted.add(suffix); }
             else suffix.add(P);
         }
-        if (sl == 3 && !Asum.is_inf()) { for (int i = 0; i < 3; ++i) Asum = Asum.dbl(); Usum.add(Asum); }
-        if (!weighted.is_inf()) for (int i = 0; i < gr.chunk_log; ++i) weighted = weighted.dbl();
+        if (sl == 3 && !Asum.is_inf()) Usum.add(xyzz_times_pow2(Asum, 3));
+        weighted = xyzz_times_pow2(weighted, (uint32_t)gr.chunk_log);
         Usum.add(weighted); Usum.add(suffix);
         V[w] = Usum;
     };
@@ -1320,20 +1352,18 @@
         });
         XYZZ<F> Usum = XYZZ<F>::inf(), suffix = XYZZ<F>::inf(), seg_weighted = XYZZ<F>::inf(), weighted = XYZZ<F>::inf();
         for (int sg = nseg - 1; sg >= 0; --sg) { Usum.add(Us[sg]); weighted.add(Wt[sg]); suffix.add(Ps[sg]); if (sg >= 1) seg_weighted.add(suffix); }
-        if (!seg_weighted.is_inf()) for (int i = 0; i < 4; ++i) seg_weighted = seg_weighted.dbl();
-        weighted.add(seg_weighted);
-        if (!weighted.is_inf()) for (int i = 0; i < gr.chunk_log; ++i) weighted = weighted.dbl();
+        weighted.add(xyzz_times_pow2(seg_weighted, 4));
+        weighted = xyzz_times_pow2(weighted, (uint32_t)gr.chunk_log);
         Usum.add(weighted); Usum.add(suffix);
         return Usum;
     }
     host_parallel_for((int)W, window);
     XYZZ<F> acc = XYZZ<F>::inf();
     for (int w = (int)W - 1; w >= 0; --w) {
-        if (!acc.is_inf()) for (uint32_t i = 0; i < g.c * g.ws; ++i) acc = acc.dbl();
+        acc = xyzz_times_pow2(acc, g.c * g.ws);
         acc.add(V[w]);
     }
-    if (!acc.is_inf()) for (uint32_t i = 0; i < g.c * g.w0; ++i) acc = acc.dbl();
-    return acc;
+    return xyzz_times_pow2(acc, g.c * g.w0);
 }
 
 static constexpr int COMBINE_THREADS = 256;
@@ -1401,7 +1431,7 @@
     size_t nblk = (total + 1024 * SCAN_ITEMS - 1) / (1024 * SCAN_ITEMS);
     if (nblk > 1024) { set_error("msm: too many buckets for the block scan"); return ZKG_ERROR; }
     if (job->digits.reserve(std::max<size_t>(1, n * g.W) * 4) || job->hist.reserve((size_t)g.W * S * g.B * 4) || job->counts.reserve(total * 4) ||
-        job->offsets.reserve((total + 1) * 4) || job->scan_sums.reserve(1024 * 4) || job->class_hist.reserve((HEAVY_T_MAX + 2) * 4) ||
+        job->offsets.reserve((total + 1) * 4) || job->scan_sums.reserve(1024 * 4) || job->class_hist.reserve((CLASS_HIST_COPIES + 1) * (HEAVY_T_MAX + 2) * 4) ||
         job->order.reserve(total * 4) || job->sorted.reserve(std::max<size_t>(1, n * g.W) * 4)) return ZKG_ERROR;
     uint32_t *digits = job->digits.as<uint32_t>(), *hist = job->hist.as<uint32_t>(), *counts = job->counts.as<uint32_t>(),
              *offsets = job->offsets.as<uint32_t>(), *sums = job->scan_sums.as<uint32_t>(), *chist = job->class_hist.as<uint32_t>();
@@ -1412,15 +1442,15 @@
     {
         ZeroList zl{};
         int k = 0;
-        zl.p[k] = chist; zl.words[k++] = HEAVY_T_MAX + 2;
+        zl.p[k] = chist; zl.words[k++] = (CLASS_HIST_COPIES + 1) * (HEAVY_T_MAX + 2);
         for (MsmGroup &gr : job->group) if (gr.nsets) {
             if (gr.heavy_counters.reserve(8 * MSM_MAX_SETS)) return ZKG_ERROR;
             zl.p[k] = gr.heavy_counters.as<uint32_t>(); zl.words[k++] = 2 * MSM_MAX_SETS;
         }
         if (two_pass) {
             const uint32_t nbins = g.W << cbits;
-            if (job->rx_meta.reserve((3 * (size_t)nbins + 8) * 4)) return ZKG_ERROR;
-            zl.p[k] = job->rx_meta.as<uint32_t>(); zl.words[k++] = 3 * nbins + 8;
+            if (job->rx_meta.reserve((2 * (size_t)nbins + g.W) * 4)) return ZKG_ERROR;
+            zl.p[k] = job->rx_meta.as<uint32_t>(); zl.words[k++] = 2 * nbins + g.W;
         }
         const dim3 dg((unsigned)((n0 + 255) / 256));
         const bool four = !d_gather && (n0 & 3) == 0 && g0.w0 == 0 && g0.ws == 1 && g0.W == g0.Wt;
@@ -1439,20 +1469,20 @@
     }
     if (two_pass) {
         const uint32_t fbits = g.c - 1 - cbits, CB = 1u << cbits, nbins = g.W * CB, S1 = (uint32_t)((n + RX_SLICE - 1) / RX_SLICE);
-        if (job->rx_tmp.reserve(n * g.W * 4) || job->rx_meta.reserve((3 * (size_t)nbins + 8) * 4)) return ZKG_ERROR;
-        uint32_t *cnt = job->rx_meta.as<uint32_t>(), *base = cnt + nbins, *cursor = base + nbins + 1, *tmp = job->rx_tmp.as<uint32_t>();
-        hipLaunchKernelGGL(k_rx_count, dim3(S1, g.W), dim3(1024), 0, s, digits, n, fbits, cbits, cnt);
-        hipLaunchKernelGGL(k_rx_scan, dim3(1), dim3(1024), 0, s, cnt, nbins, base, cursor, offsets + total);
+        if (job->rx_tmp.reserve(n * g.W * 4)) return ZKG_ERROR;
+        uint32_t *cnt = job->rx_meta.as<uint32_t>(), *cursor = cnt + nbins, *wtot = cursor + nbins, *tmp = job->rx_tmp.as<uint32_t>();
+        const size_t fine_lds = (RX_FINE_MAX + 3 * (1u << fbits)) * 4;
+        hipLaunchKernelGGL(k_rx_count, dim3(S1, g.W), dim3(1024), 0, s, digits, n, fbits, cbits, cnt, wtot);
         static const int wg_env = getenv("ZKG_SORT_WG") ? atoi(getenv("ZKG_SORT_WG")) : 0;
         const bool half = (wg_env ? wg_env == 512 : job->sort_stream != nullptr) && fbits <= 9;
         if (half) {
             const uint32_t S2 = (uint32_t)((n + 512 * RX_PER_THREAD - 1) / (512 * RX_PER_THREAD));
-            hipLaunchKernelGGL(k_rx_scatter<512>, dim3(S2, g.W), dim3(512), (512 * RX_PER_THREAD + 4 * RX_MAX_CB + 8) * 4, s, digits, n, fbits, cbits, base, cursor, tmp);
-            hipLaunchKernelGGL(k_rx_fine<512>, dim3(CB, g.W), dim3(512), (RX_FINE_MAX + 3 * (1u << fbits)) * 4, s, tmp, fbits, cbits, g.B, base, counts, offsets,
+            hipLaunchKernelGGL(k_rx_scatter<512>, dim3(S2, g.W), dim3(512), (512 * RX_PER_THREAD + 4 * RX_MAX_CB + 8) * 4, s, digits, n, fbits, cbits, cnt, wtot, g.W, cursor, tmp, offsets + total);
+            hipLaunchKernelGGL(k_rx_fine<512>, dim3(CB, g.W), dim3(512), fine_lds, s, tmp, fbits, cbits, g.B, cnt, wtot, counts, offsets, total, chist,
                                job->sorted.as<uint32_t>());
         } else {
-            hipLaunchKernelGGL(k_rx_scatter<1024>, dim3(S1, g.W), dim3(1024), (RX_SLICE + 4 * RX_MAX_CB + 8) * 4, s, digits, n, fbits, cbits, base, cursor, tmp);
-            hipLaunchKernelGGL(k_rx_fine<1024>, dim3(CB, g.W), dim3(1024), (RX_FINE_MAX + 3 * (1u << fbits)) * 4, s, tmp, fbits, cbits, g.B, base, counts, offsets,
+            hipLaunchKernelGGL(k_rx_scatter<1024>, dim3(S1, g.W), dim3(1024), (RX_SLICE + 4 * RX_MAX_CB + 8) * 4, s, digits, n, fbits, cbits, cnt, wtot, g.W, cursor, tmp, offsets + total);
+            hipLaunchKernelGGL(k_rx_fine<1024>, dim3(CB, g.W), dim3(1024), fine_lds, s, tmp, fbits, cbits, g.B, cnt, wtot, counts, offsets, total, chist,
                                job->sorted.as<uint32_t>());
         }
     } else {
@@ -1462,10 +1492,9 @@
     hipLaunchKernelGGL(k_scan_sums, dim3(1), dim3(1024), 0, s, sums, (uint32_t)nblk, offsets + total);
     hipLaunchKernelGGL(k_scan_apply, dim3((unsigned)nblk), dim3(1024), 0, s, offsets, sums, total);
     hipLaunchKernelGGL(k_place, dim3(S, g.W), dim3(SORT_THREADS), g.B * 4, s, digits, n, g.B, S, slice_len, hist, offsets, job->sorted.as<uint32_t>());
-    }
     hipLaunchKernelGGL(k_class_hist, dim3((unsigned)((total + 1023) / 1024)), dim3(1024), 0, s, counts, offsets, total, chist);
-    hipLaunchKernelGGL(k_class_scan, dim3(1), dim3(1024), 0, s, chist, offsets, total);
-    hipLaunchKernelGGL(k_order_place, dim3((unsigned)((total + 1023) / 1024)), dim3(1024), 0, s, counts, offsets, total, chist, job->order.as<uint32_t>());
+    }
+    hipLaunchKernelGGL(k_order_place, dim3((unsigned)((total + 1023) / 1024)), dim3(1024), 0, s, counts, offsets, total, chist, chist + CLASS_HIST_COPIES * (HEAVY_T_MAX + 2), job->order.as<uint32_t>());
     if (hipGetLastError() != hipSuccess) { set_error("msm sort launch failed"); return ZKG_ERROR; }
     return ZKG_OK;
 }
```

After: 55.24, median of 6. 1.02x the previous value.
